# Kloudy-Sky/openintel

Hardware: AMD Instinct MI355X
Metric: queries/sec + p50 latency, 10M-post/768-d hybrid BM25+cosine+RRF top-100 (higher is better)
Workload: dtype f32

## Files before the change

openintel_amd/csrc/api.hip:

```cpp
#include <algorithm>
#include <cstdlib>
#include <cstring>
#include <set>

#include "oi_internal.h"

static thread_local char g_err[512] = "";

void oi_set_error(const char *fmt, ...) {
    va_list ap;
    va_start(ap, fmt);
    vsnprintf(g_err, sizeof(g_err), fmt, ap);
    va_end(ap);
}

__attribute__((constructor)) static void oi_ask_for_more_hw_queues() { (void)setenv("GPU_MAX_HW_QUEUES", "8", 0); }

extern "C" const char *oi_last_error(void) { return g_err; }
extern "C" int oi_abi_version(void) { return OI_ABI_VERSION; }

int oi_dyn_lds(oi_ctx *ctx, const void *kernel, size_t bytes) {
    static std::mutex mu;
    static std::set<std::pair<const void *, int>> done;
    std::lock_guard<std::mutex> g(mu);
    const auto key = std::make_pair(kernel, ctx->device);
    if (done.count(key)) return OI_OK;
    OI_HIP_CHECK(hipFuncSetAttribute(kernel, hipFuncAttributeMaxDynamicSharedMemorySize, (int)bytes));
    done.insert(key);
    return OI_OK;
}

std::atomic<uint64_t> g_oi_ws_epoch{1};

int DevBuf::ensure(size_t bytes) {
    if (bytes <= cap && p) return OI_OK;
    if (borrowed) { oi_set_error("internal: a borrowed buffer cannot grow"); return OI_ERR_STATE; }
    g_oi_ws_epoch.fetch_add(1);
    if (p) {
        (void)hipFree(p);
        p = nullptr;
        cap = 0;
    }
    size_t want = (bytes + 255) & ~(size_t)255;
    if (want == 0) want = 256;
    OI_HIP_CHECK(hipMalloc(&p, want));
    cap = want;
    return OI_OK;
}
void DevBuf::release() {
    if (p) g_oi_ws_epoch.fetch_add(1);
    if (p && !borrowed) (void)hipFree(p);
    p = nullptr;
    cap = 0;
    borrowed = false;
}

int PinBuf::ensure(size_t bytes) {
    if (bytes <= cap) return OI_OK;
    release();
    const size_t want = (bytes + 4095) & ~(size_t)4095;
    if (hipHostMalloc(&p, want, hipHostMallocDefault) == hipSuccess) {
        pinned = true;
    } else {
        (void)hipGetLastError();
        p = aligned_alloc(4096, want);
        pinned = false;
        if (!p) { oi_set_error("host staging buffer: out of memory (%zu bytes)", want); return OI_ERR_HIP; }
    }
    cap = want;
    return OI_OK;
}
void PinBuf::release() {
    if (p) {
        if (pinned) (void)hipHostFree(p);
        else free(p);
    }
    p = nullptr;
    cap = 0;
}

void oi_ctx::prof_begin(const char *tag) {
    ProfSpan s;
    if (hipEventCreateWithFlags(&s.a, hipEventDisableSystemFence) != hipSuccess ||
        hipEventCreateWithFlags(&s.b, hipEventDisableSystemFence) != hipSuccess) return;
    (void)hipEventRecord(s.a, stream);
    prof[tag].push_back(s);
}
void oi_ctx::prof_end(const char *tag) {
    auto it = prof.find(tag);
    if (it == prof.end() || it->second.empty()) return;
    (void)hipEventRecord(it->second.back().b, stream);
}

extern "C" int oi_profile_reset(oi_ctx *ctx, int enable) {
    if (!ctx) { oi_set_error("null ctx"); return OI_ERR_INVALID_ARG; }
    std::lock_guard<std::mutex> g(ctx->mu);
    for (auto &kv : ctx->prof)
        for (auto &s : kv.second) { (void)hipEventDestroy(s.a); (void)hipEventDestroy(s.b); }
    ctx->prof.clear();
    for (const char *runs : {"volume_runs", "summary_runs", "groups_runs", "share_runs"}) {
        auto vr = ctx->ws.find(runs);
        if (vr != ctx->ws.end() && vr->second.p) (void)hipMemsetAsync(vr->second.p, 0, 16, ctx->stream);
    }
    ctx->prof_enabled = enable == 2 ? 2 : (enable != 0 ? 1 : 0);
    return OI_OK;
}

extern "C" int oi_profile_read(oi_ctx *ctx, const char *kernel_tag, double *total_ms_out, uint64_t *launches_out) {
    if (!ctx || !kernel_tag) { oi_set_error("null argument"); return OI_ERR_INVALID_ARG; }
    std::lock_guard<std::mutex> g(ctx->mu);
    OI_HIP_CHECK(hipStreamSynchronize(ctx->stream));
    double total = 0.0;
    uint64_t n = 0;
    if (strncmp(kernel_tag, "flagword", 8) == 0) {
        uint32_t w[4] = {0, 0, 0, 0};
        DevBuf &st = ctx->buf("state_flag");
        if (st.p) OI_HIP_CHECK(hipMemcpy(w, st.p, 16, hipMemcpyDeviceToHost));
        if (total_ms_out) *total_ms_out = (double)w[(kernel_tag[8] - '0') & 3];
        if (launches_out) *launches_out = 0;
        return OI_OK;
    }
    if (strcmp(kernel_tag, "graph_replays") == 0 || strcmp(kernel_tag, "graph_captures") == 0) {
        if (total_ms_out) *total_ms_out = 0.0;
        if (launches_out) *launches_out = kernel_tag[6] == 'r' ? ctx->graph_replays : ctx->graph_captures;
        return OI_OK;
    }
    if (strcmp(kernel_tag, "spec_state") == 0) {
        oi_spec_take_failure(ctx);
        if (total_ms_out) *total_ms_out = (double)ctx->spec_failures;
        if (launches_out) *launches_out = ctx->spec_searches;
        return OI_OK;
    }
    if (strcmp(kernel_tag, "screen_gate") == 0) {
        uint32_t g = 0;
        if (ctx->last_screen_gate) OI_HIP_CHECK(hipMemcpy(&g, ctx->last_screen_gate, 4, hipMemcpyDeviceToHost));
        if (total_ms_out) *total_ms_out = ctx->last_screen_gate ? (double)g : -1.0;
        if (launches_out) *launches_out = 0;
        return OI_OK;
    }
    if (strcmp(kernel_tag, "screen_width") == 0) {
        if (total_ms_out) *total_ms_out = (double)ctx->last_screen_wgs;
        if (launches_out) *launches_out = (uint64_t)ctx->num_cus;
        return OI_OK;
    }
    if (strcmp(kernel_tag, "volume_state") == 0 || strcmp(kernel_tag, "summary_state") == 0 || strcmp(kernel_tag, "groups_state") == 0 ||
        strcmp(kernel_tag, "share_state") == 0) {
        uint32_t w[4] = {0, 0, 0, 0};
        auto vs = ctx->ws.find(kernel_tag);
        if (vs != ctx->ws.end() && vs->second.p) OI_HIP_CHECK(hipMemcpy(w, vs->second.p, 16, hipMemcpyDeviceToHost));
        if (total_ms_out) *total_ms_out = (double)w[2];
        if (launches_out) *launches_out = (w[0] ? 1u : 0u) | (w[1] ? 2u : 0u);
        return OI_OK;
    }
    auto it = ctx->prof.find(kernel_tag);
    if (it != ctx->prof.end())
        for (auto &s : it->second) {
            float ms = 0.f;
            if (hipEventElapsedTime(&ms, s.a, s.b) == hipSuccess) { total += ms; ++n; }
        }
    const char *family = strcmp(kernel_tag, "volume_exact") == 0 ? "volume" : strcmp(kernel_tag, "summary_exact") == 0 ? "summary"
                       : strcmp(kernel_tag, "groups_exact") == 0 ? "groups" : strcmp(kernel_tag, "share_exact") == 0 ? "share" : nullptr;
    if (family) {
        uint32_t runs = 0;
        auto vr = ctx->ws.find(std::string(family) + "_runs");
        if (vr != ctx->ws.end() && vr->second.p) OI_HIP_CHECK(hipMemcpy(&runs, vr->second.p, 4, hipMemcpyDeviceToHost));
        auto fb = ctx->prof.find(std::string(family) + "_fallback");
        if (runs && fb != ctx->prof.end()) {
            for (auto &s : fb->second) {
                float ms = 0.f;
                if (hipEventElapsedTime(&ms, s.a, s.b) == hipSuccess) total += ms;
            }
            n += runs;
        }
    }
    if (total_ms_out) *total_ms_out = total;
    if (launches_out) *launches_out = n;
    return OI_OK;
}

#define OI_MAX_GRAPHS 32

static void graph_free(GraphEntry &e) {
    if (e.exec) (void)hipGraphExecDestroy(e.exec);
    if (e.graph) (void)hipGraphDestroy(e.graph);
    e.exec = nullptr;
    e.graph = nullptr;
}

static void graphs_purge(oi_ctx *ctx, uint64_t index_uid) {
    for (size_t i = 0; i < ctx->graphs.size();)
        if (index_uid == 0 || ctx->graphs[i].key[0] == index_uid) {
            graph_free(ctx->graphs[i]);
            ctx->graphs.erase(ctx->graphs.begin() + (long)i);
        } else ++i;
}

template <class F> static int run_captured(oi_ctx *ctx, const uint64_t (&key)[10], F &&body) {
    if (!ctx->use_graphs || ctx->prof_enabled || !ctx->stream) return body();
    const uint64_t epoch = g_oi_ws_epoch.load();
    GraphEntry *e = nullptr;
    for (auto &g : ctx->graphs)
        if (memcmp(g.key, key, sizeof(key)) == 0) { e = &g; break; }
    if (!e) {
        if (ctx->graphs.size() >= OI_MAX_GRAPHS) {
            size_t lru = 0;
            for (size_t i = 1; i < ctx->graphs.size(); ++i)
                if (ctx->graphs[i].last_use < ctx->graphs[lru].last_use) lru = i;
            OI_HIP_CHECK(hipStreamSynchronize(ctx->stream));
            graph_free(ctx->graphs[lru]);
            ctx->graphs.erase(ctx->graphs.begin() + (long)lru);
        }
        ctx->graphs.emplace_back();
        e = &ctx->graphs.back();
        memcpy(e->key, key, sizeof(key));
        e->last_use = ++ctx->graph_clock;
        const int rc = body();
        e->epoch = g_oi_ws_epoch.load();
        return rc;
    }
    e->last_use = ++ctx->graph_clock;
    if (e->epoch != epoch) {
        OI_HIP_CHECK(hipStreamSynchronize(ctx->stream));
        graph_free(*e);
        e->state = 0;
        const int rc = body();
        e->epoch = g_oi_ws_epoch.load();
        return rc;
    }
    if (e->state == 2) return body();
    if (e->state == 1) {
        OI_HIP_CHECK(hipGraphLaunch(e->exec, ctx->stream));
        ++ctx->graph_replays;
        return OI_OK;
    }
    if (hipStreamBeginCapture(ctx->stream, hipStreamCaptureModeRelaxed) != hipSuccess) {
        (void)hipGetLastError();
        e->state = 2;
        return body();
    }
    const int rc = body();
    hipGraph_t g = nullptr;
    const hipError_t end = hipStreamEndCapture(ctx->stream, &g);
    if (rc != OI_OK || end != hipSuccess || !g || g_oi_ws_epoch.load() != epoch) {
        (void)hipGetLastError();
        if (g) (void)hipGraphDestroy(g);
        e->state = 2;
        if (rc != OI_OK) return rc;
        return body();
    }
    hipGraphExec_t x = nullptr;
    if (hipGraphInstantiate(&x, g, nullptr, nullptr, 0) != hipSuccess || !x) {
        (void)hipGetLastError();
        (void)hipGraphDestroy(g);
        e->state = 2;
        return body();
    }
    e->graph = g;
    e->exec = x;
    e->state = 1;
    ++ctx->graph_captures;
    OI_HIP_CHECK(hipGraphLaunch(e->exec, ctx->stream));
    return OI_OK;
}

extern "C" int oi_set_graph_replay(oi_ctx *ctx, int enable) {
    if (!ctx) { oi_set_error("null ctx"); return OI_ERR_INVALID_ARG; }
    std::lock_guard<std::mutex> g(ctx->mu);
    ctx->use_graphs = enable != 0;
    if (!ctx->use_graphs) {
        OI_HIP_CHECK(hipSetDevice(ctx->device));
        OI_HIP_CHECK(hipStreamSynchronize(ctx->stream));
        graphs_purge(ctx, 0);
    }
    return OI_OK;
}

extern "C" int oi_create(int device_ordinal, oi_ctx **out) {
    if (!out) { oi_set_error("oi_create: out is null"); return OI_ERR_INVALID_ARG; }
    *out = nullptr;
    int n = 0;
    if (hipGetDeviceCount(&n) != hipSuccess || n <= 0) {
        oi_set_error("oi_create: no HIP device visible (this library has no CPU fallback)");
        return OI_ERR_NO_DEVICE;
    }
    OI_REQUIRE(device_ordinal >= 0 && device_ordinal < n, "oi_create: device %d of %d", device_ordinal, n);
    OI_HIP_CHECK(hipSetDevice(device_ordinal));
    hipDeviceProp_t prop;
    OI_HIP_CHECK(hipGetDeviceProperties(&prop, device_ordinal));
    if (strncmp(prop.gcnArchName, "gfx950", 6) != 0) {
        oi_set_error("oi_create: device %d is %s; this library is built for gfx950 only", device_ordinal,
                     prop.gcnArchName);
        return OI_ERR_NO_DEVICE;
    }
    oi_ctx *c = new oi_ctx();
    c->device = device_ordinal;
    c->num_cus = prop.multiProcessorCount > 0 ? prop.multiProcessorCount : 256;
    c->stream = nullptr;
    if (const char *m = getenv("OI_COSINE_MODE"))
        c->cosine_mode = strcmp(m, "split") == 0 ? OI_COSINE_SPLIT : strcmp(m, "exact") == 0 ? OI_COSINE_EXACT
                         : strcmp(m, "screen-copy") == 0 ? OI_COSINE_SCREEN_COPY
                         : strcmp(m, "screen-stream") == 0 ? OI_COSINE_SCREEN_STREAM : OI_COSINE_SCREEN;
    if (hipEventCreateWithFlags(&c->ev_fork, hipEventDisableTiming) != hipSuccess) c->ev_fork = nullptr;
    if (hipEventCreateWithFlags(&c->ev_join, hipEventDisableTiming) != hipSuccess) c->ev_join = nullptr;
    *out = c;
    return OI_OK;
}

extern "C" int oi_create_like(oi_ctx *like, oi_ctx **out) {
    if (!out) { oi_set_error("oi_create_like: out is null"); return OI_ERR_INVALID_ARG; }
    *out = nullptr;
    if (!like) { oi_set_error("null ctx"); return OI_ERR_INVALID_ARG; }
    OI_CHECK(oi_create(like->device, out));
    std::lock_guard<std::mutex> g(like->mu);
    (*out)->cosine_mode = like->cosine_mode;
    (*out)->overlap_legs = like->overlap_legs;
    (*out)->speculate = like->speculate;
    (*out)->use_graphs = like->use_graphs;
    return OI_OK;
}

static void ctx_release(oi_ctx *ctx) {
    if (ctx->refs.fetch_sub(1) != 1) return;
    (void)hipSetDevice(ctx->device);
    if (ctx->side_stream) { (void)hipStreamSynchronize(ctx->side_stream); (void)hipStreamDestroy(ctx->side_stream); }
    if (ctx->ev_fork) (void)hipEventDestroy(ctx->ev_fork);
    if (ctx->ev_join) (void)hipEventDestroy(ctx->ev_join);
    oi_profile_reset(ctx, 0);
    graphs_purge(ctx, 0);
    for (auto &kv : ctx->ws) kv.second.release();
    ctx->pin_in.release();
    ctx->pin_out.release();
    if (ctx->spec_fail_host) (void)hipHostFree(ctx->spec_fail_host);
    delete ctx;
}

extern "C" void oi_destroy(oi_ctx *ctx) {
    if (!ctx) return;
    {
        std::lock_guard<std::mutex> g(ctx->mu);
        (void)hipSetDevice(ctx->device);
        (void)hipStreamSynchronize(ctx->stream);
        if (ctx->refs.load() > 1) ctx->stream = nullptr;
    }
    ctx_release(ctx);
}

extern "C" int oi_workspace_bytes(oi_ctx *ctx, uint64_t *device_bytes, uint64_t *pinned_bytes) {
    if (!ctx) { oi_set_error("null ctx"); return OI_ERR_INVALID_ARG; }
    std::lock_guard<std::mutex> g(ctx->mu);
    uint64_t d = 0;
    for (auto &kv : ctx->ws)
        if (!kv.second.borrowed) d += kv.second.cap;
    if (device_bytes) *device_bytes = d;
    if (pinned_bytes) *pinned_bytes = (ctx->pin_in.pinned ? ctx->pin_in.cap : 0) + (ctx->pin_out.pinned ? ctx->pin_out.cap : 0);
    return OI_OK;
}

extern "C" int oi_set_stream(oi_ctx *ctx, void *hip_stream) {
    if (!ctx) { oi_set_error("null ctx"); return OI_ERR_INVALID_ARG; }
    std::lock_guard<std::mutex> g(ctx->mu);
    ctx->stream = reinterpret_cast<hipStream_t>(hip_stream);
    return OI_OK;
}

extern "C" int oi_set_cosine_mode(oi_ctx *ctx, int mode) {
    if (!ctx) { oi_set_error("null ctx"); return OI_ERR_INVALID_ARG; }
    OI_REQUIRE(mode == OI_COSINE_EXACT || mode == OI_COSINE_SPLIT || mode == OI_COSINE_SCREEN || mode == OI_COSINE_SCREEN_COPY ||
                   mode == OI_COSINE_SCREEN_STREAM,
               "oi_set_cosine_mode: unknown mode %d", mode);
    std::lock_guard<std::mutex> g(ctx->mu);
    ctx->cosine_mode = mode;
    return OI_OK;
}

extern "C" int oi_set_overlap(oi_ctx *ctx, int enable) {
    if (!ctx) { oi_set_error("null ctx"); return OI_ERR_INVALID_ARG; }
    std::lock_guard<std::mutex> g(ctx->mu);
    ctx->overlap_legs = enable != 0;
    return OI_OK;
}

extern "C" int oi_set_screen_speculation(oi_ctx *ctx, int enable) {
    if (!ctx) { oi_set_error("null ctx"); return OI_ERR_INVALID_ARG; }
    std::lock_guard<std::mutex> g(ctx->mu);
    ctx->speculate = enable != 0;
    ctx->spec_skip = ctx->spec_backoff = 0;
    return OI_OK;
}

static int check_overflow_locked(oi_ctx *ctx) {
    DevBuf &st = ctx->buf("state_flag");
    if (!st.p) return OI_OK;
    uint32_t f = 0;
    OI_HIP_CHECK(hipMemcpyAsync(&f, st.p, sizeof(f), hipMemcpyDeviceToHost, ctx->stream));
    OI_HIP_CHECK(hipStreamSynchronize(ctx->stream));
    if (f) {
        OI_HIP_CHECK(hipMemsetAsync(st.p, 0, 16, ctx->stream));
        oi_set_error("internal candidate pool overflowed");
        return OI_ERR_OVERFLOW;
    }
    return OI_OK;
}

extern "C" int oi_synchronize(oi_ctx *ctx) {
    if (!ctx) { oi_set_error("null ctx"); return OI_ERR_INVALID_ARG; }
    std::lock_guard<std::mutex> g(ctx->mu);
    OI_HIP_CHECK(hipSetDevice(ctx->device));
    OI_HIP_CHECK(hipStreamSynchronize(ctx->stream));
    return check_overflow_locked(ctx);
}

extern "C" int oi_lexicon_analyze_device(oi_ctx *ctx, const uint8_t *d_blob, const uint64_t *d_offsets,
                                         uint64_t n, uint64_t blob_bytes, double *d_pol, uint8_t *d_spec) {
    if (!ctx) { oi_set_error("null ctx"); return OI_ERR_INVALID_ARG; }
    if (n == 0) return OI_OK;
    OI_REQUIRE(d_offsets && d_pol && d_spec && (d_blob || blob_bytes == 0), "lexicon: null buffer");
    std::lock_guard<std::mutex> g(ctx->mu);
    OI_HIP_CHECK(hipSetDevice(ctx->device));
    return oi_launch_lexicon(ctx, d_blob, d_offsets, n, blob_bytes, d_pol, d_spec);
}

extern "C" int oi_lexicon_summary_device(oi_ctx *ctx, const uint8_t *d_blob, const uint64_t *d_offsets, uint64_t n,
                                         uint64_t blob_bytes, const uint8_t *d_sources, double tau, double *d_pol,
                                         uint8_t *d_spec, oi_social_counters *out) {
    if (!ctx || !out) { oi_set_error("null argument"); return OI_ERR_INVALID_ARG; }
    if (n == 0) { memset(out, 0, sizeof(*out)); return OI_OK; }
    OI_REQUIRE(d_offsets && (d_blob || blob_bytes == 0), "lexicon summary: null buffer");
    std::lock_guard<std::mutex> g(ctx->mu);
    OI_HIP_CHECK(hipSetDevice(ctx->device));
    return oi_launch_lexicon_fused(ctx, d_blob, d_offsets, n, blob_bytes, d_pol, d_spec, d_sources, tau, out);
}

extern "C" int oi_lexicon_analyze(oi_ctx *ctx, const uint8_t *blob, const uint64_t *offsets, uint64_t n,
                                  double *pol_out, uint8_t *spec_out) {
    if (!ctx) { oi_set_error("null ctx"); return OI_ERR_INVALID_ARG; }
    if (n == 0) return OI_OK;
    OI_REQUIRE(offsets && pol_out && spec_out, "lexicon: null buffer");
    OI_REQUIRE(offsets[0] == 0, "lexicon: offsets[0] must be 0");
    const uint64_t bytes = offsets[n];
    OI_REQUIRE(blob || bytes == 0, "lexicon: null text blob");
    std::lock_guard<std::mutex> g(ctx->mu);
    OI_HIP_CHECK(hipSetDevice(ctx->device));
    hipStream_t st = ctx->stream;
    const size_t off_o = (bytes + 15) & ~(size_t)15, in_bytes = off_o + sizeof(uint64_t) * (n + 1);
    const size_t out_bytes = sizeof(double) * n + n;
// ... 1620 lines not shown
```

openintel_amd/csrc/cosine_screen_i8.hip:

```cpp
#include <algorithm>
#include <cmath>
#include <cstdlib>
#include <type_traits>

#include "oi_device.h"
#include "oi_internal.h"
#include "oi_screen_stage.h"
#include "oi_lds_dma.h"

typedef int i8s_i32x4 __attribute__((ext_vector_type(4)));
typedef int i8s_i32x16 __attribute__((ext_vector_type(16)));
typedef float i8s_f32x2 __attribute__((ext_vector_type(2)));
template <int N>
struct i8s_ivec {
    typedef int type __attribute__((ext_vector_type(N)));
};

#define I8S_TILE_ROWS 32
#define I8S_SLOT_BYTES (I8S_TILE_ROWS * 128)
#define I8S_META_BYTES 256
#define I8S_PAD_ROWS 64

size_t oi_screen_i8_meta_offset(uint64_t n, uint32_t dim) { return ((size_t)n * dim + 255) & ~(size_t)255; }
size_t oi_screen_i8_bytes(uint64_t n, uint32_t dim) {
    return oi_screen_i8_meta_offset(n, dim) + 8 * ((size_t)n + I8S_PAD_ROWS) + 256;
}

__global__ __launch_bounds__(256) void i8s_make_kernel(const float *__restrict__ rows, uint64_t n, uint32_t dim,
                                                       const uint32_t *__restrict__ long_bitmap, uint32_t *__restrict__ out_i8,
                                                       float *__restrict__ meta, uint32_t *__restrict__ emax_bits) {
    const uint32_t lane = threadIdx.x & 63;
    const uint64_t wave = ((uint64_t)blockIdx.x * blockDim.x + threadIdx.x) >> 6;
    const uint64_t n_waves = ((uint64_t)gridDim.x * blockDim.x) >> 6;
    const uint32_t nv = dim >> 2;
    float best = 0.f;
    for (uint64_t r = wave; r < n; r += n_waves) {
        const float4 *x = reinterpret_cast<const float4 *>(rows + r * dim);
        float4 v[3];
        float amax = 0.f;
#pragma unroll
        for (int u = 0; u < 3; ++u) {
            const uint32_t j = lane + 64u * u;
            v[u] = j < nv ? x[j] : make_float4(0.f, 0.f, 0.f, 0.f);
            amax = fmaxf(amax, fmaxf(fmaxf(fabsf(v[u].x), fabsf(v[u].y)), fmaxf(fabsf(v[u].z), fabsf(v[u].w))));
        }
#pragma unroll
        for (int o = 32; o > 0; o >>= 1) amax = fmaxf(amax, __shfl_xor(amax, o, OI_WAVE));
        const float s = amax / 127.f;
        double e2 = 0.0;
#pragma unroll
        for (int u = 0; u < 3; ++u) {
            const uint32_t j = lane + 64u * u;
            const float xs[4] = {v[u].x, v[u].y, v[u].z, v[u].w};
            uint32_t packed = 0;
#pragma unroll
            for (int c = 0; c < 4; ++c) {
                float t = s > 0.f ? rintf(xs[c] / s) : 0.f;
                t = fminf(127.f, fmaxf(-127.f, t));
                const int iv = (int)t;
                const double e = (double)s * (double)iv - (double)xs[c];
                e2 += j < nv ? e * e : 0.0;
                packed |= ((uint32_t)iv & 0xFFu) << (8 * c);
            }
            if (j < nv) out_i8[r * nv + j] = packed;
        }
        e2 = oi_wave_sum(e2);
        const float er = (float)sqrt(e2) * 1.00000095367431640625f;
        if (lane == 0) {
            meta[2 * r] = s;
            meta[2 * r + 1] = er;
        }
        const bool is_long = long_bitmap && ((long_bitmap[r >> 5] >> (r & 31)) & 1u);
        if (!is_long) best = fmaxf(best, er);
    }
    if (lane == 0) atomicMax(emax_bits, __float_as_uint(best));
}

int oi_launch_make_screen_i8(oi_ctx *ctx, const float *rows, uint64_t n, uint32_t dim, const uint32_t *long_bitmap, uint8_t *out) {
    OI_REQUIRE(oi_cosine_screen_supported(dim), "int8 screening copy: dim %u not instantiated (384, 768)", dim);
    const size_t mo = oi_screen_i8_meta_offset(n, dim);
    OI_HIP_CHECK(hipMemsetAsync(out + mo, 0, 8 * ((size_t)n + I8S_PAD_ROWS) + 256, ctx->stream));
    if (n == 0) return OI_OK;
    uint64_t blocks = (n + 3) / 4;
    const uint64_t cap = (uint64_t)ctx->num_cus * 8;
    if (blocks > cap) blocks = cap;
    float *meta = reinterpret_cast<float *>(out + mo);
    hipLaunchKernelGGL(i8s_make_kernel, dim3((uint32_t)blocks), dim3(256), 0, ctx->stream, rows, n, dim, long_bitmap,
                       reinterpret_cast<uint32_t *>(out), meta, reinterpret_cast<uint32_t *>(meta + 2 * (n + I8S_PAD_ROWS)));
    OI_HIP_CHECK(hipGetLastError());
    return OI_OK;
}

#define I8S_NORM_LIMIT 1.0e15f
#define I8S_QNORM_MIN 1.0e-12f
__device__ __forceinline__ void i8s_stage_query_row(const float *__restrict__ q, uint32_t row, uint32_t n_queries, uint32_t n_padded, uint32_t dim,
                                                    const uint32_t *__restrict__ max_norm_bits, const uint32_t *__restrict__ emax_bits,
                                                    int8_t *__restrict__ qi8, float *__restrict__ qf, uint32_t *gate) {
    const uint32_t lane = threadIdx.x & 63;
    const bool real = row < n_queries;
    float amax = 0.f;
    bool fin = true;
    for (uint32_t k = lane; k < dim; k += 64) {
        const float f = real ? q[(uint64_t)row * dim + k] : 0.f;
        fin = fin && (f - f == 0.f);
        amax = fmaxf(amax, fabsf(f));
    }
#pragma unroll
    for (int o = 32; o > 0; o >>= 1) amax = fmaxf(amax, __shfl_xor(amax, o, OI_WAVE));
    fin = __builtin_amdgcn_ballot_w64(!fin) == 0ull;
    const float a = fin ? amax / 127.f : 0.f;
    double qn2 = 0.0, en2 = 0.0;
    for (uint32_t k = lane; k < dim; k += 64) {
        const float f = real ? q[(uint64_t)row * dim + k] : 0.f;
        float h = 0.f, l = 0.f;
        if (a > 0.f) {
            const float t = f / a;
            h = fminf(127.f, fmaxf(-127.f, rintf(t)));
            l = fminf(127.f, fmaxf(-127.f, rintf((t - h) * 128.f)));
        }
        const double qh = (double)a * ((double)h + (double)l * 0.0078125);
        qn2 += qh * qh;
        en2 += (qh - (double)f) * (qh - (double)f);
        qi8[(uint64_t)row * dim + k] = (int8_t)(int)h;
        qi8[((uint64_t)n_padded + row) * dim + k] = (int8_t)(int)l;
    }
    qn2 = oi_wave_sum(qn2);
    en2 = oi_wave_sum(en2);
    if (lane == 0) {
        const float up = 1.00000095367431640625f;
        const float qn = (float)sqrt(qn2) * up, en = (float)sqrt(en2) * up;
        const float X = __uint_as_float(max_norm_bits[0]), em = __uint_as_float(*emax_bits);
        const bool ok = fin && amax > 0.f && qn < I8S_NORM_LIMIT && qn >= I8S_QNORM_MIN && X < I8S_NORM_LIMIT && em < I8S_NORM_LIMIT;
        const float rnd = 3.814697265625e-06f + (float)dim * 2.384185791015625e-07f;
        const float cq = 1.001f * (X * en + rnd * (X + em) * (qn + en)) + 1.0e-27f;
        const float m2 = 2.002f * (em * qn + cq);
        qf[row] = ok ? a : 0.f;
        qf[n_padded + row] = ok ? qn : 0.f;
        qf[2 * n_padded + row] = ok ? cq : 0.f;
        qf[3 * n_padded + row] = ok || !real ? m2 : __builtin_inff();
        if (real && !ok) *gate = 1u;
    }
}
__global__ __launch_bounds__(256) void i8s_stage_kernel(const float *__restrict__ q, uint32_t n_queries, uint32_t n_padded, uint32_t dim,
                                                        const uint32_t *__restrict__ max_norm_bits, const uint32_t *__restrict__ emax_bits,
                                                        int8_t *__restrict__ qi8, float *__restrict__ qf, uint32_t *gate) {
    const uint32_t wave = (blockIdx.x * blockDim.x + threadIdx.x) >> 6, n_waves = (gridDim.x * blockDim.x) >> 6;
    for (uint32_t row = wave; row < n_padded; row += n_waves) {
        i8s_stage_query_row(q, row, n_queries, n_padded, dim, max_norm_bits, emax_bits, qi8, qf, gate);
    }
}

__global__ __launch_bounds__(256) void i8s_stage_both_kernel(const float *__restrict__ q, uint32_t n_queries, uint32_t n_padded, uint32_t dim,
                                                             const uint32_t *__restrict__ max_norm_bits, const uint32_t *__restrict__ emax_bits,
                                                             int8_t *__restrict__ qi8, float *__restrict__ qf, uint16_t *__restrict__ q_bf16,
                                                             float *__restrict__ eps2, uint32_t *gate) {
    const uint32_t wave = (blockIdx.x * blockDim.x + threadIdx.x) >> 6, n_waves = (gridDim.x * blockDim.x) >> 6;
    for (uint32_t row = wave; row < n_padded; row += n_waves) {
        i8s_stage_query_row(q, row, n_queries, n_padded, dim, max_norm_bits, emax_bits, qi8, qf, gate);
        pf_stage_query_row(q, row, n_queries, dim, max_norm_bits, q_bf16, eps2, gate);
    }
}

int oi_launch_screen_stage_i8(oi_ctx *ctx, const float *d_queries, uint32_t n_queries, uint32_t dim, const uint32_t *max_norm_bits,
                              const uint8_t *i8_copy, uint64_t n_rows, int8_t *qi8, float *qf, uint32_t *gate, uint16_t *q_bf16,
                              float *eps2) {
    const uint32_t n_padded = (n_queries + 31u) & ~31u;
    if (n_padded == 0) return OI_OK;
    const uint32_t *emax = reinterpret_cast<const uint32_t *>(i8_copy + oi_screen_i8_meta_offset(n_rows, dim)) + 2 * (n_rows + I8S_PAD_ROWS);
    if (q_bf16)
        hipLaunchKernelGGL(i8s_stage_both_kernel, dim3((n_padded + 3) / 4), dim3(256), 0, ctx->stream, d_queries, n_queries, n_padded, dim,
                           max_norm_bits, emax, qi8, qf, q_bf16, eps2, gate);
    else
        hipLaunchKernelGGL(i8s_stage_kernel, dim3((n_padded + 3) / 4), dim3(256), 0, ctx->stream, d_queries, n_queries, n_padded, dim,
                           max_norm_bits, emax, qi8, qf, gate);
    OI_HIP_CHECK(hipGetLastError());
    return OI_OK;
}

__device__ __forceinline__ void i8s_issue_piece(const oi_u32x4 &srd, uint32_t voff, uint32_t soff, uint32_t lds_dst) {
#ifdef I8S_NO_DMA
    (void)srd; (void)voff; (void)soff; (void)lds_dst;
#else
    oi_dma_piece(srd, voff, soff, lds_dst);
#endif
}
__device__ __forceinline__ void i8s_issue_meta(const oi_u32x4 &srd, uint32_t voff, uint32_t lds_dst) {
#ifdef I8S_NO_DMA
    (void)srd; (void)voff; (void)lds_dst;
#else
    uint32_t keep;
    const uint32_t d = __builtin_amdgcn_readfirstlane(lds_dst);
    asm volatile(
        "s_mov_b32 %0, m0\n\t"
        "s_mov_b32 m0, %3\n\t"
        "s_nop 0\n\t"
        "buffer_load_dword %1, %2, 0 offen " OI_DMA_NT "lds\n\t"
        "s_mov_b32 m0, %0"
        : "=&s"(keep)
        : "v"(voff), "s"(srd), "s"(d)
        : "memory");
#endif
}

template <int D, int NQT, int NBUF, bool FILT>
__global__ __launch_bounds__(256, 1) void cosine_i8_screen(
    const uint8_t *__restrict__ rows, const float *__restrict__ meta, uint64_t row_begin, uint64_t row_end,
    const int8_t *__restrict__ qhi, const int8_t *__restrict__ qlo,
    const float *__restrict__ qf, uint32_t qf_stride, uint32_t n_queries, uint32_t doc_id_base, uint64_t *pools, uint32_t *seg_cnt,
    uint32_t seg_cnt_stride, const uint32_t *tau_keys, uint64_t pool_stride, uint32_t carry_cap, uint32_t seg_cap, uint32_t *overflow,
    const uint4 *__restrict__ filt, const uint2 *__restrict__ attrs) {
    constexpr int NKC = D / 128;
    constexpr int P = NBUF - 1;
    constexpr int KSTEPS = D / 32;
    constexpr uint32_t RING = NBUF * I8S_SLOT_BYTES;
    static_assert(D % 128 == 0 && P >= 2 && P <= 2 * NKC, "unsupported ring depth for this D");
    constexpr uint32_t QLO_LDS = NQT * KSTEPS * 64 * 16;
    static_assert(NQT * KSTEPS * 4 <= 200, "the hi query block must fit the register file");
    static_assert(4 * RING + 4 * 2 * I8S_META_BYTES + 256 + OI_STAGE_LDS + QLO_LDS <= 160 * 1024, "LDS");

    extern __shared__ __attribute__((aligned(1024))) unsigned char smem[];
    unsigned char *ring = smem;
    unsigned char *meta_lds = smem + 4 * RING;
    uint32_t *seg_fill = reinterpret_cast<uint32_t *>(smem + 4 * RING + 8 * I8S_META_BYTES);
    unsigned char *stage_base = smem + 4 * RING + 8 * I8S_META_BYTES + 256;
    unsigned char *qlo_lds = stage_base + OI_STAGE_LDS;

    OI_CLAIM_WHOLE_SIMD();
    const uint32_t tid = threadIdx.x, lane = tid & 63;
    const uint32_t w = __builtin_amdgcn_readfirstlane(tid >> 6);
    const uint32_t li = lane & 31, lh = lane >> 5;
    uint64_t *stage_keys = reinterpret_cast<uint64_t *>(stage_base) + w * OI_STAGE;
    uint32_t *stage_q = reinterpret_cast<uint32_t *>(stage_base + 4 * OI_STAGE * 8) + w * OI_STAGE;
    uint32_t st_head = 0, st_n = 0;

    i8s_i32x4 qh[NQT][KSTEPS];
#pragma unroll
    for (int t = 0; t < NQT; ++t)
#pragma unroll
        for (int s = 0; s < KSTEPS; ++s)
            qh[t][s] = *reinterpret_cast<const i8s_i32x4 *>(qhi + (uint64_t)(32 * t + li) * D + 32 * s + 16 * lh);
    for (uint32_t c = tid; c < (uint32_t)(NQT * KSTEPS * 64); c += 256) {
        const uint32_t t = c / (KSTEPS * 64), s = (c / 64) % KSTEPS, l = c % 64;
        *reinterpret_cast<i8s_i32x4 *>(qlo_lds + c * 16) =
            *reinterpret_cast<const i8s_i32x4 *>(qlo + (uint64_t)(32 * t + (l & 31)) * D + 32 * s + 16 * (l >> 5));
    }
    float qa[NQT], qn[NQT], cq[NQT], tc[NQT];
#pragma unroll
    for (int t = 0; t < NQT; ++t) {
        const uint32_t q = 32u * t + li;
        const bool real = q < n_queries;
        const uint32_t k = real ? tau_keys[q] : 0xFFFFFFFFu;
        const float tau = k <= 0x007FFFFFu ? -__builtin_inff() : oi_key_f32(k);
        qa[t] = real ? qf[q] * 0.0078125f : 0.f;
        qn[t] = real ? qf[qf_stride + q] : 0.f;
        cq[t] = real ? qf[2 * qf_stride + q] : 0.f;
        const float m2 = real ? qf[3 * qf_stride + q] : 0.f;
        const float T = m2 < __builtin_inff() ? (tau + m2) - (fabsf(tau) + m2) * 9.5367431640625e-07f : -__builtin_inff();
        tc[t] = T - cq[t];
    }
    if (tid < 32 * NQT) seg_fill[tid] = 0;
#ifdef I8S_NO_DMA
    for (uint32_t i = tid; i < (4 * RING + 8 * I8S_META_BYTES) / 4; i += 256) reinterpret_cast<uint32_t *>(smem)[i] = 0u;
#endif
    __syncthreads();

    const uint64_t n_rows = row_end - row_begin;
    const uint64_t n_tiles = (n_rows + I8S_TILE_ROWS - 1) / I8S_TILE_ROWS;
    const uint64_t first = (uint64_t)blockIdx.x * 4 + w, stride = (uint64_t)gridDim.x * 4;
    const uint64_t my_nt = first < n_tiles ? (n_tiles - first + stride - 1) / stride : 0;
    uint64_t *my_seg = pools + carry_cap + (uint64_t)blockIdx.x * seg_cap;

    if (my_nt) {
        uint32_t voff[4];
#pragma unroll
        for (int m = 0; m < 4; ++m) {
            const uint32_t prow = 8 * m + (lane >> 3);
            voff[m] = prow * (uint32_t)D + (((lane & 7) ^ ((prow >> 1) & 7)) << 4);
        }
        const uint32_t ring_w = oi_lds_addr(ring) + w * RING;
        const unsigned char *ring_rd = ring + w * RING;
        const uint32_t meta_w = oi_lds_addr(meta_lds) + w * 2 * I8S_META_BYTES;
        const unsigned char *meta_rd = meta_lds + w * 2 * I8S_META_BYTES;
        uint32_t frag_off[4];
#pragma unroll
        for (int g = 0; g < 4; ++g) frag_off[g] = li * 128 + (((2 * g + lh) ^ ((li >> 1) & 7)) << 4);

        auto tile_row0 = [&](uint64_t ti) { return row_begin + (first + ti * stride) * (uint64_t)I8S_TILE_ROWS; };
        auto tile_srd = [&](uint64_t ti) {
            const uint64_t r0 = tile_row0(ti < my_nt ? ti : 0);
            return oi_make_srd(rows + r0 * D, ti < my_nt ? (row_end - r0) * (uint64_t)D : 0ull);
        };
        auto issue_meta = [&](uint64_t ti) {
            const uint64_t r0 = tile_row0(ti);
            i8s_issue_meta(oi_make_srd(meta + 2 * r0, (row_end - r0) * 8ull), lane * 4u, meta_w + (uint32_t)(ti & 1) * I8S_META_BYTES);
        };
        oi_u32x4 s0 = tile_srd(0), s1 = tile_srd(1), s2 = tile_srd(2);
        __builtin_amdgcn_s_waitcnt(0x0F70);
        oi_static_for<0, P>([&](auto j_) {
            constexpr int j = decltype(j_)::value;
            constexpr int tj = j / NKC, kj = j % NKC;
#pragma unroll
            for (int m = 0; m < 4; ++m)
                i8s_issue_piece(tj == 0 ? s0 : (tj == 1 ? s1 : s2), voff[m], kj * 128, ring_w + j * I8S_SLOT_BYTES + m * 1024);
        });
        issue_meta(0);
        uint32_t rd_off = 0, wr_off = (NBUF - 1) * I8S_SLOT_BYTES;
        auto lo_frag = [&](int t, int s) {
            return *reinterpret_cast<const i8s_i32x4 *>(qlo_lds + ((t * KSTEPS + s) * 64 + lane) * 16);
        };
        i8s_i32x4 b_cur[NQT];
#ifndef I8S_NO_MFMA
#pragma unroll
        for (int t = 0; t < NQT; ++t) b_cur[t] = lo_frag(t, 0);
#endif

        oi_wait_vm<4 * (P - 1)>();
        i8s_i32x4 a_cur = *reinterpret_cast<const i8s_i32x4 *>(ring_rd + frag_off[0]);

        constexpr int NS = 16 * NQT;
        constexpr int RPK = KSTEPS >= 20 ? 1 : 2;
        constexpr int NSL = 16 / RPK, T0 = 4;
        static_assert(T0 + NSL <= KSTEPS, "the tile test does not fit the span");
        static_assert(4 * NKC + 4 >= 4 * (P - 1) - 1, "the ring's wait in k-step 3 must retire the previous tile's metadata");
        typename i8s_ivec<NS>::type S;
#pragma unroll
        for (int i = 0; i < NS; ++i) S[i] = 0;
        i8s_i32x16 ah[NQT], al[NQT];
        i8s_f32x2 md_cur[RPK];
#pragma unroll
        for (int u = 0; u < RPK; ++u) md_cur[u] = i8s_f32x2{0.f, 0.f};
        const uint32_t lh32 = 32u * lh;
        auto meta_row = [&](const unsigned char *mt, int r) {
            return *reinterpret_cast<const i8s_f32x2 *>(mt + lh32 + ((r & 3) + 8 * (r >> 2)) * 8);
        };
        float cap_sc = 0.f, cap_er = 0.f;
        auto test_row = [&](int t, int r, const i8s_f32x2 md) -> uint32_t {
            const float sc = oi_mul_unpacked((float)S[16 * t + r], oi_mul_unpacked(md[0], qa[t]));
            const bool pass = sc >= oi_fma_unpacked(-md[1], qn[t], tc[t]);
            cap_sc = pass ? sc : cap_sc;
            cap_er = pass ? md[1] : cap_er;
            return pass ? 1u << (16 * t + r) : 0u;
        };

        for (uint64_t ti = 0;; ++ti) {
            const bool live = ti < my_nt;
            const unsigned char *mt = meta_rd + (uint32_t)((ti + 1) & 1) * I8S_META_BYTES;
            uint32_t m = 0;
            if (live) {
#pragma unroll
                for (int t = 0; t < NQT; ++t)
#pragma unroll
                    for (int r = 0; r < 16; ++r) { ah[t][r] = 0; al[t][r] = 0; }

                oi_static_for<0, NKC * 4>([&](auto gi_) {
                    constexpr int gi = decltype(gi_)::value;
                    constexpr int kc = gi / 4, g = gi % 4;
                    constexpr int sn = kc + P;
                    constexpr int tn = sn / NKC, kn = sn % NKC;
                    i8s_i32x4 a_nxt;
                    if constexpr (g < 3) {
                        a_nxt = *reinterpret_cast<const i8s_i32x4 *>(ring_rd + rd_off + frag_off[g + 1]);
                    } else {
                        oi_wait_vm<4 * (P - 1) - 1>();
                        const uint32_t nx_off = rd_off + I8S_SLOT_BYTES == RING ? 0u : rd_off + I8S_SLOT_BYTES;
                        a_nxt = *reinterpret_cast<const i8s_i32x4 *>(ring_rd + nx_off + frag_off[0]);
                    }
                    i8s_f32x2 md_nxt[RPK];
                    if constexpr (gi >= T0 - 1 && gi < T0 - 1 + NSL) {
#pragma unroll
                        for (int u = 0; u < RPK; ++u) md_nxt[u] = meta_row(mt, RPK * (gi - (T0 - 1)) + u);
                    }
#ifndef I8S_NO_MFMA
                    i8s_i32x4 b_nxt[NQT];
#pragma unroll
                    for (int t = 0; t < NQT; ++t) b_nxt[t] = lo_frag(t, (gi + 1) % KSTEPS);
#endif
                    __builtin_amdgcn_sched_barrier(0);
#pragma unroll
                    for (int t = 0; t < NQT; ++t) {
#ifndef I8S_NO_MFMA
                        ah[t] = __builtin_amdgcn_mfma_i32_32x32x32_i8(a_cur, qh[t][gi], ah[t], 0, 0, 0);
                        al[t] = __builtin_amdgcn_mfma_i32_32x32x32_i8(a_cur, b_cur[t], al[t], 0, 0, 0);
#else
                        asm volatile("" : : "v"(a_cur));
#endif
                        if constexpr (gi >= T0 && gi < T0 + NSL) if (t == 0) {
#pragma unroll
                            for (int u = 0; u < RPK; ++u)
#pragma unroll
                                for (int tt = 0; tt < NQT; ++tt) m |= test_row(tt, RPK * (gi - T0) + u, md_cur[u]);
                            asm volatile("" : "+v"(m), "+v"(cap_sc), "+v"(cap_er));
                        }
                        __builtin_amdgcn_sched_barrier(0);
                    }
#ifndef I8S_NO_MFMA
#pragma unroll
                    for (int t = 0; t < NQT; ++t) b_cur[t] = b_nxt[t];
#endif
                    if constexpr (gi >= T0 - 1 && gi < T0 - 1 + NSL) {
#pragma unroll
                        for (int u = 0; u < RPK; ++u) md_cur[u] = md_nxt[u];
                    }
                    i8s_issue_piece(tn == 0 ? s0 : (tn == 1 ? s1 : s2), voff[g], kn * 128, ring_w + wr_off + g * 1024);
                    if constexpr (g == 3) {
                        wr_off = rd_off;
                        rd_off = rd_off + I8S_SLOT_BYTES == RING ? 0u : rd_off + I8S_SLOT_BYTES;
                    }
                    a_cur = a_nxt;
                });
            } else {
                oi_wait_vm<0>();
#pragma unroll
                for (int r = 0; r < 16; ++r) {
                    const i8s_f32x2 md = meta_row(mt, r);
#pragma unroll
                    for (int t = 0; t < NQT; ++t) m |= test_row(t, r, md);
                }
            }

            const uint64_t row0 = tile_row0(ti ? ti - 1 : 0);
            if (ti == 0) m = 0u;
            const uint32_t m_tested = m;
            if (row_end - row0 < (uint64_t)I8S_TILE_ROWS) {
                const uint32_t left = (uint32_t)(row_end - row0);
#pragma unroll
                for (int r = 0; r < 16; ++r)
                    if ((uint32_t)((r & 3) + 8 * (r >> 2)) + 4u * lh >= left) m &= ~(0x00010001u << r);
            }
#if defined(I8S_NO_DMA) || defined(I8S_NO_MFMA) || defined(I8S_NO_APPEND)
            if (seg_cap != 0xFFFFFFFFu) m = 0u;
#endif
            if (__builtin_amdgcn_ballot_w64(m != 0u) != 0ull) {
                if constexpr (FILT) m = oi_filter_tile<NQT>(m, filt, attrs, row0, lh, li);
                static_assert(64u <= OI_STAGE - OI_STAGE_FLUSH, "a tile of one pair per lane must fit the staging ring");
                if (__builtin_amdgcn_ballot_w64((m_tested & (m_tested - 1u)) != 0u) == 0ull) {
                    const uint64_t has = __builtin_amdgcn_ballot_w64(m != 0u);
                    if (m != 0u) {
                        const uint32_t bit = (uint32_t)__builtin_ctz(m), r = bit & 15u;
                        const bool t1 = NQT > 1 && bit >= 16u;
                        const uint32_t rit = (r & 3) + 8 * (r >> 2) + 4 * lh;
                        const float low = cap_sc - fmaf(cap_er, t1 ? qn[NQT - 1] : qn[0], t1 ? cq[NQT - 1] : cq[0]);
                        const uint32_t below = __builtin_amdgcn_mbcnt_hi((uint32_t)(has >> 32), __builtin_amdgcn_mbcnt_lo((uint32_t)has, 0u));
                        const uint32_t idx = (st_head + st_n + below) & (OI_STAGE - 1);
                        stage_keys[idx] = oi_rank_key(low, doc_id_base + ((uint32_t)row0 + rit));
                        stage_q[idx] = (t1 ? 32u : 0u) + li;
                    }
                    st_n += (uint32_t)__builtin_popcountll(has);
                    while (st_n >= OI_STAGE_FLUSH) {
                        OI_STAGE_FLUSH_TO_POOL(OI_STAGE_FLUSH);
                    }
                } else {
                    const uint32_t cnt = (uint32_t)__builtin_popcount(m);
                    const uint32_t incl = oi_wave_incl_scan(cnt);
                    const uint32_t total = (uint32_t)__builtin_amdgcn_readlane((int)incl, 63);
                    const uint32_t any = oi_wave_or(m);
                    auto lower_key = [&](int t, uint32_t r) -> uint64_t {
                        const uint32_t rit = (r & 3) + 8 * (r >> 2) + 4 * lh;
                        const i8s_f32x2 md = *reinterpret_cast<const i8s_f32x2 *>(mt + rit * 8);
                        const float sc = (float)S[16 * t + r] * (md[0] * qa[t]);
                        return oi_rank_key(sc - fmaf(md[1], qn[t], cq[t]), doc_id_base + ((uint32_t)row0 + rit));
                    };
                    if (total <= OI_STAGE - OI_STAGE_FLUSH) {
                        uint32_t idx = st_head + st_n + incl - cnt;
#pragma unroll
                        for (int t = 0; t < NQT; ++t)
                            for (uint32_t wd = (any >> (16 * t)) & 0xFFFFu; wd; wd &= wd - 1) {
                                const uint32_t r = (uint32_t)__builtin_ctz(wd);
                                if (m & (1u << (16 * t + r))) {
                                    stage_keys[idx & (OI_STAGE - 1)] = lower_key(t, r);
                                    stage_q[idx & (OI_STAGE - 1)] = 32u * t + li;
                                    ++idx;
                                }
                            }
                        st_n += total;
                        while (st_n >= OI_STAGE_FLUSH) {
                            OI_STAGE_FLUSH_TO_POOL(OI_STAGE_FLUSH);
                        }
                    } else {
                        uint32_t pos[NQT];
#pragma unroll
                        for (int t = 0; t < NQT; ++t)
                            pos[t] = atomicAdd(&seg_fill[32u * t + li], (uint32_t)__builtin_popcount((m >> (16 * t)) & 0xFFFFu));
#pragma unroll
                        for (int t = 0; t < NQT; ++t) {
                            uint64_t *dst = my_seg + (uint64_t)(32u * t + li) * pool_stride;
                            for (uint32_t wd = (any >> (16 * t)) & 0xFFFFu; wd; wd &= wd - 1) {
                                const uint32_t r = (uint32_t)__builtin_ctz(wd);
                                if (m & (1u << (16 * t + r))) {
                                    if (pos[t] < seg_cap) dst[pos[t]] = lower_key(t, r);
                                    else *overflow = 1u;
                                    ++pos[t];
                                }
                            }
                        }
                    }
                }
            }
            if (!live) break;
#pragma unroll
            for (int t = 0; t < NQT; ++t)
#pragma unroll
                for (int r = 0; r < 16; ++r) S[16 * t + r] = ah[t][r] * 128 + al[t][r];
            if (ti + 1 < my_nt) issue_meta(ti + 1);
            s0 = s1;
            s1 = s2;
            s2 = tile_srd(ti + 3);
        }
        if (st_n) {
            OI_STAGE_FLUSH_TO_POOL(st_n);
        }
        oi_wait_vm<0>();
    }
    __syncthreads();
    if (tid < 32 * NQT && tid < n_queries) {
        const uint32_t c = seg_fill[tid];
        seg_cnt[(uint64_t)tid * seg_cnt_stride + blockIdx.x] = c < seg_cap ? c : seg_cap;
    }
}

template <int D, int NQT, int NBUF, bool FILT>
static int launch_i8_screen_k(oi_ctx *ctx, const uint8_t *rows, const float *meta, uint64_t row_begin, uint64_t row_end, const int8_t *qhi,
                              const int8_t *qlo, const float *qf, uint32_t qf_stride, uint32_t nq, uint32_t doc_id_base, const PoolView &p) {
    constexpr size_t smem = 4 * NBUF * I8S_SLOT_BYTES + 8 * I8S_META_BYTES + 256 + OI_STAGE_LDS + NQT * (D / 32) * 64 * 16;
    OI_CHECK(oi_dyn_lds(ctx, reinterpret_cast<const void *>(cosine_i8_screen<D, NQT, NBUF, FILT>), (size_t)(smem)));
    hipLaunchKernelGGL((cosine_i8_screen<D, NQT, NBUF, FILT>), dim3(p.n_segs), dim3(256), smem, ctx->stream, rows, meta, row_begin, row_end,
                       qhi, qlo, qf, qf_stride, nq, doc_id_base, p.keys, p.seg_cnt, p.seg_cnt_stride, p.tau_keys, p.stride, p.carry_cap,
                       p.seg_cap, p.overflow, p.filt, p.attrs);
    OI_HIP_CHECK(hipGetLastError());
    return OI_OK;
}
template <int D, int NQT, int NBUF>
static int launch_i8_screen(oi_ctx *ctx, const uint8_t *rows, const float *meta, uint64_t row_begin, uint64_t row_end, const int8_t *qhi,
                            const int8_t *qlo, const float *qf, uint32_t qf_stride, uint32_t nq, uint32_t doc_id_base, const PoolView &p) {
    return p.filt ? launch_i8_screen_k<D, NQT, NBUF, true>(ctx, rows, meta, row_begin, row_end, qhi, qlo, qf, qf_stride, nq, doc_id_base, p)
                  : launch_i8_screen_k<D, NQT, NBUF, false>(ctx, rows, meta, row_begin, row_end, qhi, qlo, qf, qf_stride, nq, doc_id_base, p);
}

int oi_launch_cosine_screen_i8_chunk(oi_ctx *ctx, const uint8_t *i8_copy, uint64_t n_rows_total, uint64_t row_begin, uint64_t row_end,
                                     uint32_t dim, const int8_t *qi8, const float *qf, uint32_t n_queries, uint32_t doc_id_base,
                                     PoolView &pool, uint32_t wgs) {
    OI_REQUIRE(oi_cosine_screen_supported(dim), "cosine screen (int8): dim %u not instantiated (384, 768)", dim);
    OI_REQUIRE(row_end <= n_rows_total, "cosine screen (int8): rows past the copy");
    const uint64_t chunk_rows = row_end > row_begin ? row_end - row_begin : 0;
    if (wgs) oi_cosine_screen_geometry(ctx, chunk_rows, wgs, &pool.n_segs, &pool.seg_cap);
    else oi_cosine_screen_geometry(ctx, chunk_rows, &pool.n_segs, &pool.seg_cap);
    OI_REQUIRE(pool.n_segs <= pool.seg_cnt_stride && pool.carry_cap + (uint64_t)pool.n_segs * pool.seg_cap <= pool.stride,
               "cosine screen (int8): chunk does not fit the candidate pool");
    if (row_end <= row_begin || n_queries == 0) return OI_OK;
    const float *meta = reinterpret_cast<const float *>(i8_copy + oi_screen_i8_meta_offset(n_rows_total, dim));
    const uint32_t np = (n_queries + 31u) & ~31u;
    ProfScope ps(ctx, "cosine");
    for (uint32_t q0 = 0; q0 < n_queries; q0 += 64) {
        const uint32_t nq_here = std::min(64u, n_queries - q0);
        const PoolView p = pool.for_queries(q0);
        const int8_t *qhi = qi8 + (uint64_t)q0 * dim, *qlo = qi8 + ((uint64_t)np + q0) * dim;
        const float *qfp = qf + q0;
        const bool two = nq_here > 32;
        if (dim == 768) {
            if (two) OI_CHECK((launch_i8_screen<768, 2, 6>(ctx, i8_copy, meta, row_begin, row_end, qhi, qlo, qfp, np, nq_here, doc_id_base, p)));
            else OI_CHECK((launch_i8_screen<768, 1, 6>(ctx, i8_copy, meta, row_begin, row_end, qhi, qlo, qfp, np, nq_here, doc_id_base, p)));
        } else {
            if (two) OI_CHECK((launch_i8_screen<384, 2, 6>(ctx, i8_copy, meta, row_begin, row_end, qhi, qlo, qfp, np, nq_here, doc_id_base, p)));
            else OI_CHECK((launch_i8_screen<384, 1, 6>(ctx, i8_copy, meta, row_begin, row_end, qhi, qlo, qfp, np, nq_here, doc_id_base, p)));
        }
    }
    return OI_OK;
}

__device__ __forceinline__ float i8s_bf16_lo(uint32_t w) { return __uint_as_float(w << 16); }
__device__ __forceinline__ float i8s_bf16_hi(uint32_t w) { return __uint_as_float(w & 0xFFFF0000u); }
__global__ __launch_bounds__(256) void pf_rescreen_kernel(const uint16_t *__restrict__ copy, uint64_t n_rows, uint32_t dim,
                                                          uint32_t doc_id_base, const uint16_t *__restrict__ qb, uint64_t *pools,
                                                          const uint32_t *__restrict__ cnt, uint64_t stride, uint32_t cap) {
    const uint32_t q = blockIdx.y, lane = threadIdx.x & 63;
    const uint32_t wave = (blockIdx.x * blockDim.x + threadIdx.x) >> 6, n_waves = (gridDim.x * blockDim.x) >> 6;
    uint32_t c = cnt[q];
    c = c < cap ? c : cap;
    uint64_t *keys = pools + (uint64_t)q * stride;
    const uint32_t nvec = dim >> 3;
    const uint4 *qv = reinterpret_cast<const uint4 *>(qb + (uint64_t)q * dim);
    for (uint32_t i0 = wave * 4u; i0 < c; i0 += n_waves * 4u) {
        uint32_t doc[4];
        const uint4 *x[4];
        float a[4];
#pragma unroll
        for (int u = 0; u < 4; ++u) {
            const uint32_t i = i0 + u < c ? i0 + u : c - 1u;
            doc[u] = oi_rank_key_doc(keys[i]);
            const uint64_t r = (uint64_t)(doc[u] - doc_id_base);
            x[u] = reinterpret_cast<const uint4 *>(copy + (r < n_rows ? r : 0) * dim);
            a[u] = 0.f;
        }
        for (uint32_t v = lane; v < nvec; v += 64) {
            const uint4 yv = qv[v];
            uint4 xv[4];
#pragma unroll
            for (int u = 0; u < 4; ++u) xv[u] = oi_load_stream(x[u] + v);
#pragma unroll
            for (int u = 0; u < 4; ++u) {
                const uint32_t xw[4] = {xv[u].x, xv[u].y, xv[u].z, xv[u].w}, yw[4] = {yv.x, yv.y, yv.z, yv.w};
#pragma unroll
                for (int e = 0; e < 4; ++e) {
                    a[u] = oi_fma_unpacked(i8s_bf16_lo(xw[e]), i8s_bf16_lo(yw[e]), a[u]);
                    a[u] = oi_fma_unpacked(i8s_bf16_hi(xw[e]), i8s_bf16_hi(yw[e]), a[u]);
                }
            }
        }
        float s[4];
#pragma unroll
        for (int u = 0; u < 4; ++u) s[u] = oi_wave_sum(a[u]);
#pragma unroll
        for (int u = 0; u < 4; ++u) {
            const uint64_t r = (uint64_t)(doc[u] - doc_id_base);
            const float sc = r < n_rows ? s[u] : 0.f;
            if (lane == 0 && i0 + u < c) keys[i0 + u] = oi_rank_key(sc, doc[u]);
        }
    }
}

int oi_launch_rescreen_bf16(oi_ctx *ctx, const uint16_t *copy_rows, uint64_t n_rows, uint32_t dim, uint32_t doc_id_base,
                            const uint16_t *q_bf16, uint32_t n_queries, const PoolView &pool) {
    if (n_queries == 0) return OI_OK;
    ProfScope ps(ctx, "rescreen");
    hipLaunchKernelGGL(pf_rescreen_kernel, dim3(32, n_queries), dim3(256), 0, ctx->stream, copy_rows, n_rows, dim, doc_id_base, q_bf16,
                       pool.keys, pool.carry_cnt, pool.stride, pool.carry_cap);
    OI_HIP_CHECK(hipGetLastError());
    return OI_OK;
}
```

openintel_amd/csrc/oi_internal.h:

```cpp
#pragma once

#include <hip/hip_runtime.h>

#include <cstdarg>
#include <cstdint>
#include <cstdio>
#include <cstdlib>
#include <cstring>
#include <atomic>
#include <map>
#include <mutex>
#include <string>
#include <utility>
#include <vector>

#include "openintel_hip.h"

void oi_set_error(const char *fmt, ...);

#define OI_HIP_CHECK(expr)                                                                   \
    do {                                                                                     \
        hipError_t oi_e_ = (expr);                                                           \
        if (oi_e_ != hipSuccess) {                                                           \
            oi_set_error("%s failed: %s (%s:%d)", #expr, hipGetErrorString(oi_e_), __FILE__, \
                         __LINE__);                                                          \
            return OI_ERR_HIP;                                                               \
        }                                                                                    \
    } while (0)

#define OI_CHECK(expr)              \
    do {                            \
        int oi_rc_ = (expr);        \
        if (oi_rc_ != OI_OK) return oi_rc_; \
    } while (0)

#define OI_REQUIRE(cond, ...)         \
    do {                              \
        if (!(cond)) {                \
            oi_set_error(__VA_ARGS__); \
            return OI_ERR_INVALID_ARG; \
        }                             \
    } while (0)

struct oi_ctx;
int oi_dyn_lds(oi_ctx *ctx, const void *kernel, size_t bytes);

#ifdef OI_ABLATION
inline const char *oi_ablation_env(const char *name) { return getenv(name); }
#else
inline const char *oi_ablation_env(const char *) { return nullptr; }
#endif

struct DevBuf {
    void *p = nullptr;
    size_t cap = 0;
    bool borrowed = false;
    DevBuf() = default;
    DevBuf(const DevBuf &) = delete;
    DevBuf &operator=(const DevBuf &) = delete;
    ~DevBuf() { release(); }
    int ensure(size_t bytes);
    void release();
    template <class T> T *as() const { return reinterpret_cast<T *>(p); }
};

#define OI_PINNED_STAGE_MAX ((size_t)1 << 20)
struct PinBuf {
    void *p = nullptr;
    size_t cap = 0;
    bool pinned = false;
    PinBuf() = default;
    PinBuf(const PinBuf &) = delete;
    PinBuf &operator=(const PinBuf &) = delete;
    int ensure(size_t bytes);
    void release();
    template <class T> T *as() const { return reinterpret_cast<T *>(p); }
};

struct ProfSpan {
    hipEvent_t a, b;
};

extern std::atomic<uint64_t> g_oi_ws_epoch;

struct GraphEntry {
    uint64_t key[10] = {0, 0, 0, 0, 0, 0, 0, 0, 0, 0};
    uint64_t epoch = 0, last_use = 0;
    int state = 0;
    hipGraph_t graph = nullptr;
    hipGraphExec_t exec = nullptr;
};

struct oi_ctx {
    std::atomic<int> refs{1};
    int device = 0;
    int num_cus = 256;
    hipStream_t stream = nullptr;
    hipStream_t side_stream = nullptr;
    bool side_stream_failed = false;
    hipEvent_t ev_fork = nullptr, ev_join = nullptr;
    bool overlap_legs = true;
    bool speculate = true;
    uint32_t spec_skip = 0, spec_backoff = 0;
    uint32_t *spec_fail_host = nullptr;
    uint64_t spec_searches = 0, spec_failures = 0;
    int cosine_mode = 2;
    std::mutex mu;
    std::map<std::string, DevBuf> ws;
    int prof_enabled = 0;
    const uint32_t *run_gate = nullptr;
    const uint32_t *last_screen_gate = nullptr;
    uint32_t last_screen_wgs = 0;
    std::map<std::string, std::vector<ProfSpan>> prof;
    std::vector<hipEvent_t> event_pool;
    bool use_graphs = false;
    std::vector<GraphEntry> graphs;
    uint64_t graph_clock = 0, graph_replays = 0, graph_captures = 0;

    PinBuf pin_in, pin_out;

    DevBuf &buf(const char *name) { return ws[name]; }
    void prof_begin(const char *tag);
    void prof_end(const char *tag);
};

struct ProfScope {
    oi_ctx *c;
    const char *tag;
    bool on;
    ProfScope(oi_ctx *ctx, const char *t) : c(ctx), tag(t) {
        on = c->prof_enabled == 1 || (c->prof_enabled == 2 && strcmp(t, "cosine") == 0);
        if (on) c->prof_begin(tag);
    }
    ~ProfScope() {
        if (on) c->prof_end(tag);
    }
};

#define OI_BM25_FLOOR_RANKS 4
struct oi_index {
    uint64_t uid = 0;
    std::atomic<int> refs{1};
    oi_index *src = nullptr;
    oi_ctx *ctx = nullptr;
    uint64_t n_docs = 0;
    uint32_t dim = 0, vocab = 0, doc_id_base = 0;

    float *rows = nullptr;
    bool rows_owned = false;
    uint16_t *rows_bf16 = nullptr;
    bool rows_bf16_owned = false;
    DevBuf max_row_norm;
    bool screen_ok = false;
    uint32_t n_long = 0;
    DevBuf long_list, long_bitmap;
    DevBuf screen_copy;
    int screen_copy_policy = -1;
    DevBuf screen_i8;
    DevBuf doc_attrs;
    DevBuf signals;

    bool forward_set = false, finalized = false;
    uint64_t total_tokens = 0;
    uint64_t n_postings = 0;
    uint32_t n_blocks = 0;
    uint32_t n_win = 0;
    DevBuf uniq_keys;
    DevBuf tf;
    DevBuf doc_len;
    DevBuf df_local;

    DevBuf postings;
    DevBuf cell_start;
    DevBuf idf;
    DevBuf impact_floor;
    DevBuf fwd_terms;
    DevBuf fwd_offsets;
    float avgdl = 0.f;
    uint32_t max_query_terms = 16;
    int bm25_mode = 0;
    bool is_view = false;
};

int search_lists_device(oi_index *idx, const float *d_qv, const uint32_t *d_qt, const uint32_t *d_qo, uint32_t B, uint32_t depth,
                        float *cos_s, uint32_t *cos_d, uint32_t *cos_c, float *bm_s, uint32_t *bm_d, uint32_t *bm_c,
                        const uint4 *d_filt = nullptr, const uint2 *d_attrs = nullptr);
void oi_spec_take_failure(oi_ctx *ctx);

int oi_launch_lexicon(oi_ctx *ctx, const uint8_t *d_blob, const uint64_t *d_offsets, uint64_t n,
                      uint64_t blob_bytes, double *d_pol, uint8_t *d_spec);
int oi_launch_lexicon_fused(oi_ctx *ctx, const uint8_t *d_blob, const uint64_t *d_offsets, uint64_t n, uint64_t blob_bytes,
                            double *d_pol, uint8_t *d_spec, const uint8_t *d_sources, double tau, oi_social_counters *summary);
int oi_launch_social_summary(oi_ctx *ctx, const uint8_t *d_sources, const double *d_pol,
                             const uint8_t *d_spec, uint64_t n, double tau,
                             oi_social_counters *out_host);
int oi_launch_social_summary_segmented(oi_ctx *ctx, const uint8_t *d_sources, const double *d_pol, const uint8_t *d_spec,
                                       uint64_t n, const uint64_t *d_seg, uint64_t n_seg, double tau,
                                       oi_social_counters *d_out);
int oi_launch_headline_scan(oi_ctx *ctx, const uint8_t *d_blob, const uint64_t *d_offsets, uint64_t n,
                            uint64_t blob_bytes, const uint8_t *ticker, uint64_t ticker_len,
                            const uint8_t *forms_blob, const uint32_t *form_offsets, uint32_t n_forms,
                            uint16_t *d_mask, uint64_t *d_order, uint8_t *d_about);
size_t oi_headline_params_bytes();
int oi_headline_build_params(void *dst, const uint8_t *ticker, uint64_t ticker_len, const uint8_t *forms_blob,
                             const uint32_t *form_offsets, uint32_t n_forms);
int oi_launch_headline_scan_params(oi_ctx *ctx, const uint8_t *d_blob, const uint64_t *d_offsets, uint64_t n,
                                   uint64_t blob_bytes, uint64_t text_bytes, const void *d_params, uint16_t *d_mask,
                                   uint64_t *d_order, uint8_t *d_about);
struct PoolView {
    uint64_t *keys;
    uint32_t *carry_cnt;
    uint32_t *seg_cnt;
    uint32_t *tau_keys;
    uint64_t stride;
    uint32_t carry_cap;
    uint32_t seg_cap;
    uint32_t n_segs;
    uint32_t seg_cnt_stride;
    uint32_t *overflow;
    const uint4 *filt = nullptr;
    const uint2 *attrs = nullptr;

    PoolView for_queries(uint32_t q0) const {
        PoolView p = *this;
        p.keys += (uint64_t)q0 * stride;
        p.carry_cnt += q0;
        p.seg_cnt += (uint64_t)q0 * seg_cnt_stride;
        if (p.tau_keys) p.tau_keys += q0;
        if (p.filt) p.filt += q0;
        return p;
    }
};
struct SelectExtra {
    const float *eps2 = nullptr;
    uint32_t *margin_gate = nullptr;
    const uint32_t *run_gate = nullptr;
    const uint32_t *skip_bitmap = nullptr;
    uint32_t skip_base = 0;
    uint64_t *cand = nullptr;
    uint32_t cand_cap = 0;
    const float *row_meta = nullptr;
    uint32_t meta_base = 0;
    const float *row_qn = nullptr, *row_cq = nullptr;
    uint32_t spec_rank = 0;
    uint32_t *spec_tau = nullptr, *spec_max = nullptr;
};
int oi_launch_select(oi_ctx *ctx, const PoolView &pool, uint32_t n_queries, uint32_t k, bool compact,
                     float *out_scores, uint32_t *out_docs, uint32_t *out_counts, uint32_t out_stride,
                     const SelectExtra *extra = nullptr);
int oi_launch_lists_to_pool(oi_ctx *ctx, const float *scores, const uint32_t *docs,
                            const uint32_t *counts, uint64_t shard_stride, uint64_t count_stride,
                            uint32_t n_shards, uint32_t n_queries, uint32_t depth, const PoolView &pool);
int oi_launch_rrf(oi_ctx *ctx, const uint32_t *docs_a, const uint32_t *counts_a, const uint32_t *docs_b,
                  const uint32_t *counts_b, uint32_t n_queries, uint32_t depth, uint32_t k,
                  float *scores_out, uint32_t *docs_out, uint32_t *counts_out);
int oi_launch_collapse(oi_index *idx, const float *d_scores, const uint32_t *d_docs, const uint32_t *d_counts, uint32_t n_queries,
                       uint32_t depth, float threshold, uint32_t k, float *scores_out, uint32_t *docs_out, uint32_t *counts_out,
                       uint32_t *dup_out);
int oi_launch_similar_volume(oi_index *idx, const float *d_q, uint32_t n_queries, const oi_volume_spec &spec, const uint4 *d_filt,
                             uint32_t *d_counts);
int oi_launch_volume_round_queries(oi_ctx *ctx, const float *d_q, uint64_t total, float *d_out);
int oi_launch_pack_signals(oi_ctx *ctx, const double *d_pol, const uint8_t *d_spec, const uint8_t *d_sources, uint64_t n, double tau,
                           uint2 *d_out);
int oi_launch_similar_summary(oi_index *idx, const float *d_q, uint32_t n_queries, const oi_summary_spec &spec, const float *d_thresholds,
                              const uint4 *d_filt, oi_social_counters *d_out);
int oi_launch_similar_groups(oi_index *idx, const float *d_q, uint32_t n_queries, const oi_groups_spec &spec, const float *d_thresholds,
                             const uint4 *d_filt, oi_social_counters *d_records, uint32_t *d_keys, uint32_t *d_counts,
                             uint32_t *d_qualified);
int oi_launch_similar_share(oi_index *idx, const float *d_q, uint32_t n_queries, const oi_summary_spec &spec, const float *d_thresholds,
                            const uint4 *d_filt, oi_social_counters *d_out, uint32_t *d_labels);
int oi_launch_mention_summary(oi_index *idx, const uint32_t *d_terms, const uint32_t *d_offsets, uint32_t n_queries,
                              const oi_mention_spec &spec, const uint32_t *d_min_match, const uint4 *d_filt, oi_social_counters *d_out);
int oi_launch_label_sums(oi_index *idx, const uint32_t *d_labels, uint32_t n_clusters, int64_t *d_sums, uint64_t *d_counts);
int oi_launch_centroids_from_sums(oi_ctx *ctx, const int64_t *d_sums, const uint64_t *d_counts, const float *d_previous,
                                  uint32_t n_clusters, uint32_t dim, float *d_out);
int oi_launch_fit_moved(oi_ctx *ctx, const uint32_t *d_cur, const uint32_t *d_prev, uint64_t n, uint64_t *d_out);
int oi_launch_cosine_chunk(oi_ctx *ctx, const float *rows, uint64_t row_begin, uint64_t row_end,
                           uint32_t dim, const float *d_queries_padded, uint32_t n_queries,
                           uint32_t n_queries_padded, uint32_t doc_id_base, PoolView &pool);
uint64_t oi_cosine_max_chunk_rows(const oi_ctx *ctx, uint32_t dim, uint32_t n_queries, uint64_t stride,
                                  uint32_t carry_cap);
int oi_launch_l2_normalize(oi_ctx *ctx, float *rows, uint64_t n, uint32_t dim);
bool oi_cosine_split_supported(uint32_t dim);
int oi_launch_cosine_split(oi_ctx *ctx, const float *rows, uint64_t row_begin, uint64_t row_end, uint32_t dim,
                           const float *d_queries, uint32_t nq, uint32_t doc_id_base, const PoolView &p);
bool oi_cosine_bf16_supported(uint32_t dim);
int oi_launch_cosine_bf16_chunk(oi_ctx *ctx, const uint16_t *rows, uint64_t row_begin, uint64_t row_end, uint32_t dim,
                                const float *d_queries, uint32_t n_queries, uint32_t doc_id_base, PoolView &pool);
uint32_t oi_cosine_query_padding(uint32_t n_queries);
bool oi_cosine_ksplit_supported(uint32_t dim);
bool oi_cosine_screen_supported(uint32_t dim);
inline bool oi_index_screenable(const oi_index *idx) {
    return idx->rows && !idx->rows_bf16 && idx->screen_ok && oi_cosine_screen_supported(idx->dim);
}
void oi_cosine_screen_geometry(const oi_ctx *ctx, uint64_t n_rows, uint32_t *n_segs, uint32_t *seg_cap);
void oi_cosine_screen_geometry(const oi_ctx *ctx, uint64_t n_rows, uint32_t wgs, uint32_t *n_segs, uint32_t *seg_cap);
int oi_launch_row_norm_max(oi_ctx *ctx, const float *rows, uint64_t n, uint32_t dim, uint32_t *max_bits);
int oi_launch_screen_stage(oi_ctx *ctx, const float *d_queries, uint32_t n_queries, uint32_t dim,
                           const uint32_t *max_norm_bits, uint16_t *q_bf16, float *eps2, uint32_t *gate);
int oi_launch_cosine_screen_chunk(oi_ctx *ctx, const float *rows, uint64_t row_begin, uint64_t row_end, uint32_t dim,
                                  const uint16_t *q_bf16, uint32_t n_queries, uint32_t doc_id_base, PoolView &pool);
int oi_launch_make_screen_copy(oi_ctx *ctx, const float *rows, uint64_t n, uint32_t dim, uint16_t *out);
#define OI_I8_CARRY 16384u
size_t oi_screen_i8_bytes(uint64_t n, uint32_t dim);
size_t oi_screen_i8_meta_offset(uint64_t n, uint32_t dim);
int oi_launch_make_screen_i8(oi_ctx *ctx, const float *rows, uint64_t n, uint32_t dim, const uint32_t *long_bitmap, uint8_t *out);
int oi_launch_screen_stage_i8(oi_ctx *ctx, const float *d_queries, uint32_t n_queries, uint32_t dim, const uint32_t *max_norm_bits,
                              const uint8_t *i8_copy, uint64_t n_rows, int8_t *qi8, float *qf, uint32_t *gate,
                              uint16_t *q_bf16 = nullptr, float *eps2 = nullptr);
int oi_launch_cosine_screen_i8_chunk(oi_ctx *ctx, const uint8_t *i8_copy, uint64_t n_rows_total, uint64_t row_begin, uint64_t row_end,
                                     uint32_t dim, const int8_t *qi8, const float *qf, uint32_t n_queries, uint32_t doc_id_base,
                                     PoolView &pool, uint32_t wgs = 0);
int oi_launch_rescreen_bf16(oi_ctx *ctx, const uint16_t *copy_rows, uint64_t n_rows, uint32_t dim, uint32_t doc_id_base,
                            const uint16_t *q_bf16, uint32_t n_queries, const PoolView &pool);
int oi_launch_cosine_screen_copy_chunk(oi_ctx *ctx, const uint16_t *copy_rows, uint64_t row_begin, uint64_t row_end, uint32_t dim,
                                       const uint16_t *q_bf16, uint32_t n_queries, uint32_t doc_id_base, PoolView &pool);
int oi_launch_screen_probe(oi_ctx *ctx, const float *rows, uint64_t row_begin, uint32_t n_rows, uint32_t dim,
                           const uint16_t *q_bf16, uint32_t n_queries, float *d_out);
int oi_launch_spec_threshold(oi_ctx *ctx, const PoolView &pool, uint32_t n_queries, uint32_t r, const float *eps2, uint32_t *spec_tau,
                             uint32_t *spec_max);
int oi_launch_spec_compare(oi_ctx *ctx, uint32_t n_queries, const uint32_t *tau_a, const uint32_t *max_a, const uint32_t *tau_b,
                           const uint32_t *max_b);
int oi_launch_rescore(oi_ctx *ctx, const float *rows, uint64_t n_rows, uint32_t dim, uint32_t doc_id_base,
                      const float *d_queries, uint32_t n_queries, const PoolView &in, const PoolView &out,
                      const uint32_t *extra_docs = nullptr, uint32_t n_extra = 0, const uint32_t *spec_max = nullptr,
                      const uint32_t *tau_final = nullptr, uint32_t *gate = nullptr, uint32_t *fail_host = nullptr);
#define OI_LONG_ROWS_MAX 1024u
int oi_launch_row_norm_classes(oi_ctx *ctx, const float *rows, uint64_t n, uint32_t dim, float X0, float E0, uint32_t *cls,
                               uint32_t *bitmap, uint32_t *list, uint32_t cap);
int oi_launch_cosine_ksplit(oi_ctx *ctx, const float *rows, uint64_t row_begin, uint64_t row_end, uint32_t dim,
                            const float *q, uint32_t nq, bool two_tiles, uint32_t doc_id_base, const PoolView &p);
int oi_bm25_stage_forward(oi_index *idx, const uint32_t *d_terms, const uint64_t *d_offsets);
int oi_bm25_finalize(oi_index *idx, uint64_t global_n, uint64_t global_tokens, const uint32_t *global_df_host);
void oi_bm25_scan_geometry(const oi_ctx *ctx, uint64_t n_docs, uint32_t *n_segs, uint32_t *seg_cap);
uint32_t oi_bm25_scan_pass_queries(uint32_t max_terms_per_query);
int oi_launch_bm25_scan(oi_index *idx, const uint32_t *d_q_terms, const uint32_t *d_q_offsets, uint32_t q_begin,
                        uint32_t nq, uint64_t doc_begin, uint64_t doc_end, float avgdl, bool run_setup,
                        const PoolView &pool);
uint32_t oi_bm25_wave_pass_queries(void);
int oi_launch_bm25_wave(oi_index *idx, const uint32_t *d_q_terms, const uint32_t *d_q_offsets, uint32_t q_begin,
                        uint32_t nq, const PoolView &pool, uint32_t block_begin, uint32_t block_end);
uint32_t oi_bm25_stream_pass_queries(void);
uint32_t oi_bm25_stream_seg_cap(uint32_t depth, bool first_phase);
int oi_launch_bm25_plan(oi_index *idx, const uint32_t *d_q_terms, const uint32_t *d_q_offsets, uint32_t q_begin, uint32_t nq,
                        uint32_t *state, uint64_t state_words, uint32_t depth, uint32_t tau_off, uint32_t tau_words, bool with_floors);
int oi_launch_bm25_stream(oi_index *idx, const uint32_t *d_q_terms, const uint32_t *d_q_offsets, uint32_t q_begin,
                          uint32_t nq, uint32_t depth, const PoolView &pool, uint32_t block_begin, uint32_t block_end);
int oi_launch_bm25(oi_index *idx, const uint32_t *d_q_terms, const uint32_t *d_q_offsets,
                   uint32_t n_queries, uint32_t depth, const PoolView &pool, uint32_t block_begin,
                   uint32_t block_end);

struct oi_comm {
    oi_ctx *ctx = nullptr;
    void *nccl = nullptr;
    uint32_t rank = 0, world = 1;
};
int oi_rccl_unique_id(uint8_t *id_out);
int oi_rccl_init(void **comm_out, uint32_t world, const uint8_t *id_bytes, uint32_t rank);
void oi_rccl_destroy(void *comm);
int oi_rccl_all_gather_u32(void *comm, const uint32_t *send, uint32_t *recv, size_t words, hipStream_t st);
int oi_rccl_all_reduce_sum(void *comm, void *buf, size_t count, bool u64, hipStream_t st);
```

openintel_amd/csrc/search.hip:

```cpp
#include <algorithm>

#include "oi_internal.h"

namespace {

int env_int(const char *name, int dflt, int lo) { return oi_ablation_env(name) ? std::max(lo, atoi(oi_ablation_env(name))) : dflt; }
bool env_set(const char *name) { return oi_ablation_env(name) != nullptr; }
struct Knobs {
    uint64_t first_mult = env_int("OI_FIRST_CHUNK_MULT", 1, 1), first_div = env_int("OI_FIRST_CHUNK_DIV", 1, 1);
    uint64_t growth = env_int("OI_CHUNK_GROWTH", 0, 2);
    uint64_t spec_growth = env_int("OI_SPEC_GROWTH", 128, 2), spec_first_div = env_int("OI_SPEC_FIRST_DIV", 4, 1);
    uint32_t bm25_first_div = env_int("OI_BM25_FIRST_DIV", 8, 1);
    bool screen_no_round = env_set("OI_SCREEN_NO_ROUND"), no_spec = env_set("OI_NO_SPEC"), no_overlap = env_set("OI_NO_OVERLAP");
    bool bm25_beside_last = env_set("OI_BM25_BESIDE_LAST"), screen_i8_narrow = env_set("OI_SCREEN_I8_NARROW");
    bool bm25_early = env_set("OI_BM25_EARLY"), small_gemv = env_set("OI_SMALL_BATCH_GEMV"), bm25_two_phase = env_set("OI_BM25_TWO_PHASE");
    bool exact_only = env_set("OI_COSINE_V1") || env_set("OI_SELECT_V1");
};
const Knobs &knobs() { static const Knobs k; return k; }

struct Pools { PoolView cos, bm; };
enum { BM25_TAAT = 1, BM25_SCAN = 2, BM25_WAVE = 3, BM25_STREAM = 4 };
int bm25_mode_of(const oi_index *idx) {
    static const char *mode_env = getenv("OI_BM25_MODE");
    int mode = idx->bm25_mode;
    if (mode == 0 && mode_env)
        mode = strcmp(mode_env, "scan") == 0 ? 2 : strcmp(mode_env, "taat") == 0 ? 1 : strcmp(mode_env, "wave") == 0 ? 3 : 4;
    return mode == 0 ? 4 : mode;
}
int prepare_pools(oi_ctx *ctx, uint32_t B, uint64_t cos_alloc_stride, uint64_t cos_stride, uint32_t carry_cap, uint32_t bm_blocks,
                  uint32_t depth, Pools *out, size_t extra_words, uint32_t **extra) {
    DevBuf &flag = ctx->buf("state_flag");
    if (!flag.p) {
        OI_CHECK(flag.ensure(16));
        OI_HIP_CHECK(hipMemsetAsync(flag.p, 0, 16, ctx->stream));
    }
    const uint32_t cos_segs = (uint32_t)ctx->num_cus * (B <= 8 ? 8u : 1u);
    const uint32_t bm_segs = bm_blocks ? bm_blocks : 1;
    const size_t words = (size_t)B * (2 + cos_segs + 2 + bm_segs);
    DevBuf &st = ctx->buf("pool_state");
    OI_CHECK(st.ensure(sizeof(uint32_t) * (words + extra_words)));
    OI_HIP_CHECK(hipMemsetAsync(st.p, 0, sizeof(uint32_t) * (words + extra_words), ctx->stream));
    *extra = st.as<uint32_t>() + words;
    const uint64_t bm_stride = (uint64_t)carry_cap + (uint64_t)bm_segs * depth;
    DevBuf &pc = ctx->buf("pool_cos"), &pb = ctx->buf("pool_bm");
    OI_CHECK(pc.ensure(sizeof(uint64_t) * (size_t)B * cos_alloc_stride));
    OI_CHECK(pb.ensure(sizeof(uint64_t) * (size_t)B * bm_stride));
    uint32_t *s = st.as<uint32_t>();
    uint32_t *cos_carry = s, *cos_tau = s + B, *cos_seg = s + 2 * (size_t)B;
    uint32_t *bm_carry = cos_seg + (size_t)B * cos_segs, *bm_tau = bm_carry + B, *bm_seg = bm_tau + B;
    out->cos = PoolView{pc.as<uint64_t>(), cos_carry, cos_seg, cos_tau, cos_stride, carry_cap, 0, 0, cos_segs, flag.as<uint32_t>()};
    out->bm = PoolView{pb.as<uint64_t>(), bm_carry, bm_seg, bm_tau, bm_stride, carry_cap, depth, bm_segs, bm_segs, flag.as<uint32_t>()};
    return OI_OK;
}

uint64_t oi_first_chunk_rows(uint32_t depth) {
    return std::max<uint64_t>(std::max<uint64_t>(8192, 32ull * depth) * knobs().first_mult / knobs().first_div, 2ull * depth);
}
uint64_t oi_screen_first_chunk_rows(const oi_ctx *ctx, uint32_t depth) {
    uint64_t rows = oi_first_chunk_rows(depth);
    const uint64_t round = 32ull * 4 * std::max<uint64_t>(1, (uint64_t)ctx->num_cus * 7 / 8);
    if (!knobs().screen_no_round && rows >= round) rows -= rows % round;
    return rows;
}
uint64_t oi_chunk_growth(uint32_t B) { return knobs().growth ? knobs().growth : (B <= 8 ? 16 : 8); }
uint64_t oi_chunk_end(uint64_t r, uint64_t chunk, uint64_t n, uint64_t max_chunk, uint64_t next_chunk) {
    uint64_t e = std::min(n, r + chunk);
    if (e < n && (n - e) * 4 <= (e - r) && n - r <= max_chunk) e = n;
    if (e < n && next_chunk >= max_chunk && n - e > max_chunk && n - r <= 2 * max_chunk) e = n - max_chunk;
    return e;
}

struct Chunk { uint64_t r, e; };
std::vector<Chunk> chunk_schedule(uint64_t n, uint64_t first, uint64_t growth, uint64_t max_chunk, bool stretch_first) {
    std::vector<Chunk> out;
    uint64_t chunk = first, r = 0;
    while (r < n) {
        if (chunk > max_chunk) chunk = max_chunk;
        const uint64_t e = oi_chunk_end(r, chunk, n, max_chunk, r == 0 && !stretch_first ? 0 : chunk * growth);
        out.push_back(Chunk{r, e});
        r = e;
        chunk *= growth;
    }
    return out;
}

struct Search {
    oi_index *idx; oi_ctx *ctx;
    const float *qv; const uint32_t *qt, *qo;
    uint32_t B, depth;
    float *cos_s; uint32_t *cos_d, *cos_c;
    float *bm_s; uint32_t *bm_d, *bm_c;
    const uint4 *filt; const uint2 *attrs;
};
enum class CosRoute { none, bf16, exact, screen_f32, screen_copy, screen_i8 };

struct Plan {
    CosRoute cos = CosRoute::none;
    int bm25 = BM25_STREAM;
    uint64_t cos_stride = 0, pf_stride = 0, pf_slack = 0;
    uint32_t pf_carry = 4096;
    bool spec = false;
    std::vector<Chunk> screen_chunks;
    bool overlap = false, late_fork = false, tail_fork = false;
    uint32_t screen_wgs = 0;
};
bool screened(CosRoute c) { return c == CosRoute::screen_f32 || c == CosRoute::screen_copy || c == CosRoute::screen_i8; }

Plan plan_search(const Search &s) {
    oi_index *idx = s.idx; oi_ctx *ctx = s.ctx;
    const Knobs &K = knobs();
    const uint64_t n = idx->n_docs;
    const uint32_t B = s.B, depth = s.depth, carry_cap = OI_MAX_DEPTH;
    Plan p;
    const int mode = ctx->cosine_mode;
    const bool want_copy = mode != OI_COSINE_SCREEN_STREAM && (idx->screen_copy.p != nullptr || (mode == OI_COSINE_SCREEN_COPY && !idx->is_view));
    const bool screen = (mode == OI_COSINE_SCREEN || mode == OI_COSINE_SCREEN_COPY || mode == OI_COSINE_SCREEN_STREAM) &&
                        oi_index_screenable(idx) && (B > 8 || (want_copy && !K.small_gemv)) && !K.exact_only;
    if (!s.cos_s) p.cos = CosRoute::none;
    else if (idx->rows_bf16) p.cos = CosRoute::bf16;
    else if (!screen) p.cos = CosRoute::exact;
    else if (!want_copy) p.cos = s.filt ? CosRoute::exact : CosRoute::screen_f32;
    else if (B > 8 && idx->screen_copy.p && idx->screen_i8.p) p.cos = CosRoute::screen_i8;
    else p.cos = CosRoute::screen_copy;
    p.bm25 = bm25_mode_of(idx);
    if (p.bm25 == BM25_SCAN && !(idx->fwd_terms.p && idx->total_tokens > 0)) p.bm25 = BM25_STREAM;
    if (s.filt) p.bm25 = BM25_STREAM;
    const uint64_t slack = (idx->rows_bf16 ? 128ull : 32ull) * ((uint64_t)ctx->num_cus + 1);
    const uint64_t budget = (idx->rows_bf16 ? (8ull << 30) : (13ull << 28)) / 8 / B;
    p.cos_stride = std::min<uint64_t>(carry_cap + n + slack, std::max<uint64_t>(std::min<uint64_t>(1ull << 24, budget), carry_cap + 4 * slack));
    p.pf_carry = p.cos == CosRoute::screen_i8 ? OI_I8_CARRY : 4096;
    p.pf_slack = 128ull * ((uint64_t)ctx->num_cus + 1);
    p.pf_stride = std::min<uint64_t>(p.pf_carry + n + p.pf_slack, std::max<uint64_t>(std::min<uint64_t>(1ull << 24, budget), p.pf_carry + 4 * p.pf_slack));
    uint64_t first = oi_screen_first_chunk_rows(ctx, depth), growth = oi_chunk_growth(B);
    const uint64_t pool_max = p.pf_stride - p.pf_carry - p.pf_slack;
    if (screened(p.cos) && B > 8 && !s.filt) {
        oi_spec_take_failure(ctx);
        p.spec = ctx->speculate && !K.no_spec && !ctx->use_graphs;
        if (p.spec && ctx->spec_skip) { --ctx->spec_skip; p.spec = false; }
        if (p.spec && !ctx->spec_fail_host) {
            if (hipHostMalloc(reinterpret_cast<void **>(&ctx->spec_fail_host), 64, hipHostMallocDefault) == hipSuccess) *ctx->spec_fail_host = 0;
            else { (void)hipGetLastError(); ctx->spec_fail_host = nullptr; p.spec = false; }
        }
        if (p.spec && n) {
            const uint64_t first_short = std::min<uint64_t>(n, std::max<uint64_t>(std::max<uint64_t>(8192, 8ull * depth), first / K.spec_first_div));
            if (n - first_short <= pool_max && 2 * ((3ull * depth * first_short + n - 1) / n + 12) <= depth) {
                growth = K.spec_growth;
                first = first_short;
            } else if (2 * ((3ull * depth * std::min<uint64_t>(n, first) + n - 1) / n + 12) <= depth) growth = K.spec_growth;
        }
    }
    if (screened(p.cos)) p.screen_chunks = chunk_schedule(n, first, growth, pool_max, false);
    if (s.cos_s && s.bm_s && !ctx->side_stream && !ctx->side_stream_failed && ctx->overlap_legs && !K.no_overlap) {
        if (hipStreamCreateWithFlags(&ctx->side_stream, hipStreamNonBlocking) != hipSuccess) { ctx->side_stream = nullptr; ctx->side_stream_failed = true; }
    }
    p.overlap = s.cos_s && s.bm_s && ctx->side_stream && ctx->ev_fork && ctx->ev_join && ctx->overlap_legs && !K.no_overlap;
    p.late_fork = p.overlap && !K.bm25_early && B > 8 && !p.screen_chunks.empty() &&
                  p.screen_chunks.back().e - p.screen_chunks.back().r >= (512u << 10);
    p.tail_fork = p.late_fork && p.cos == CosRoute::screen_i8 && !K.bm25_beside_last;
    if (p.cos == CosRoute::screen_i8 && !idx->is_view && (!p.overlap || p.tail_fork) && !K.screen_i8_narrow)
        p.screen_wgs = (uint32_t)std::max(1, ctx->num_cus);
    return p;
}

int bm25_stream(const Search &s, const PoolView &bm) {
    oi_index *idx = s.idx; oi_ctx *ctx = s.ctx;
    const uint32_t B = s.B, depth = s.depth, carry_cap = OI_MAX_DEPTH, nb = idx->n_blocks;
    if (nb == 0 || idx->n_postings == 0) {
        OI_HIP_CHECK(hipMemsetAsync(s.bm_c, 0, sizeof(uint32_t) * B, ctx->stream));
        return OI_OK;
    }
    const bool floors = idx->impact_floor.p != nullptr && !knobs().bm25_two_phase && !s.filt;
    const uint32_t first = floors ? nb : nb > 48 ? std::max<uint32_t>(8, nb / knobs().bm25_first_div) : nb;
    const uint32_t cap1 = oi_bm25_stream_seg_cap(depth, !floors), cap2 = oi_bm25_stream_seg_cap(depth, false);
    const uint64_t sstride = (uint64_t)carry_cap + std::max<uint64_t>((uint64_t)first * cap1, (uint64_t)nb * cap2);
    uint64_t pass = (2ull << 30) / 8 / sstride;
    pass = std::max<uint64_t>(1, std::min<uint64_t>(pass, std::min<uint32_t>(B, oi_bm25_stream_pass_queries())));
    DevBuf &sp = ctx->buf("pool_bm_stream"), &sc = ctx->buf("pool_bm_stream_state");
    OI_CHECK(sp.ensure(sizeof(uint64_t) * (size_t)pass * sstride));
    const size_t swords = (size_t)pass * (2 + nb);
    OI_CHECK(sc.ensure(sizeof(uint32_t) * swords));
    for (uint32_t q0 = 0; q0 < B; q0 += (uint32_t)pass) {
        const uint32_t nq = std::min<uint32_t>((uint32_t)pass, B - q0);
        uint32_t *w = sc.as<uint32_t>();
        OI_CHECK(oi_launch_bm25_plan(idx, s.qt, s.qo, q0, nq, w, swords, depth, (uint32_t)pass, (uint32_t)pass, floors));
        PoolView W1{sp.as<uint64_t>(), w, w + 2 * (size_t)pass, w + pass, sstride, carry_cap, cap1, first, nb, bm.overflow, s.filt, s.attrs};
        OI_CHECK(oi_launch_bm25_stream(idx, s.qt, s.qo, q0, nq, depth, W1, 0, first));
        PoolView W2 = W1;
        if (first < nb) {
            OI_CHECK(oi_launch_select(ctx, W1, nq, depth, true, nullptr, nullptr, nullptr, depth));
            W2.seg_cap = cap2; W2.n_segs = nb;
            OI_CHECK(oi_launch_bm25_stream(idx, s.qt, s.qo, q0, nq, depth, W2, first, nb));
        }
        OI_CHECK(oi_launch_select(ctx, W2, nq, depth, false, s.bm_s + (size_t)q0 * depth, s.bm_d + (size_t)q0 * depth, s.bm_c + q0, depth));
    }
    return OI_OK;
}
int bm25_wave(const Search &s, const PoolView &bm) {
    oi_index *idx = s.idx; oi_ctx *ctx = s.ctx;
    const uint32_t B = s.B, depth = s.depth, carry_cap = OI_MAX_DEPTH, nb = idx->n_blocks;
    if (nb == 0 || idx->n_postings == 0) {
        OI_HIP_CHECK(hipMemsetAsync(s.bm_c, 0, sizeof(uint32_t) * B, ctx->stream));
        return OI_OK;
    }
    const uint64_t wstride = (uint64_t)carry_cap + (uint64_t)nb * OI_BM25_BLOCK_DOCS;
    uint64_t pass = (6ull << 30) / 8 / wstride;
    pass = std::max<uint64_t>(1, std::min<uint64_t>(pass, std::min<uint32_t>(B, oi_bm25_wave_pass_queries())));
    DevBuf &wp = ctx->buf("pool_bm_wave"), &wc = ctx->buf("pool_bm_wave_state");
    OI_CHECK(wp.ensure(sizeof(uint64_t) * (size_t)pass * wstride));
    const size_t wwords = (size_t)pass * (2 + nb);
    OI_CHECK(wc.ensure(sizeof(uint32_t) * wwords));
    const uint32_t first = nb > 16 ? std::max<uint32_t>(8, nb / 8) : nb;
    for (uint32_t q0 = 0; q0 < B; q0 += (uint32_t)pass) {
        const uint32_t nq = std::min<uint32_t>((uint32_t)pass, B - q0);
        OI_HIP_CHECK(hipMemsetAsync(wc.p, 0, sizeof(uint32_t) * wwords, ctx->stream));
        uint32_t *w = wc.as<uint32_t>();
        PoolView W{wp.as<uint64_t>(), w, w + 2 * (size_t)pass, w + pass, wstride, carry_cap, OI_BM25_BLOCK_DOCS, nb, nb, bm.overflow};
        OI_CHECK(oi_launch_bm25_wave(idx, s.qt, s.qo, q0, nq, W, 0, first));
        if (first < nb) {
            OI_CHECK(oi_launch_select(ctx, W, nq, depth, true, nullptr, nullptr, nullptr, depth));
            OI_CHECK(oi_launch_bm25_wave(idx, s.qt, s.qo, q0, nq, W, first, nb));
        }
        OI_CHECK(oi_launch_select(ctx, W, nq, depth, false, s.bm_s + (size_t)q0 * depth, s.bm_d + (size_t)q0 * depth, s.bm_c + q0, depth));
    }
    return OI_OK;
}
int bm25_taat(const Search &s, const PoolView &bm) {
    const uint32_t nb = s.idx->n_blocks;
    const uint32_t first = nb > 16 ? std::max<uint32_t>(8, nb / 8) : nb;
    OI_CHECK(oi_launch_bm25(s.idx, s.qt, s.qo, s.B, s.depth, bm, 0, first));
    if (first < nb) {
        OI_CHECK(oi_launch_select(s.ctx, bm, s.B, s.depth, true, nullptr, nullptr, nullptr, s.depth));
        OI_CHECK(oi_launch_bm25(s.idx, s.qt, s.qo, s.B, s.depth, bm, first, nb));
    }
    return oi_launch_select(s.ctx, bm, s.B, s.depth, false, s.bm_s, s.bm_d, s.bm_c, s.depth);
}
int bm25_scan(const Search &s, const PoolView &bm) {
    oi_index *idx = s.idx; oi_ctx *ctx = s.ctx;
    const uint64_t n = idx->n_docs;
    const uint32_t B = s.B, depth = s.depth, carry_cap = OI_MAX_DEPTH;
    const uint32_t segs = 2u * (uint32_t)ctx->num_cus;
    const uint64_t sslack = 1024ull * (segs + 1);
    uint64_t sstride = carry_cap + std::min<uint64_t>(n, 1ull << 23) + sslack;
    const uint64_t sbudget = (4ull << 30) / 8 / B;
    if (sstride > sbudget) sstride = std::max<uint64_t>(sbudget, carry_cap + 4 * sslack);
    DevBuf &sp = ctx->buf("pool_bm_scan"), &sc = ctx->buf("pool_bm_scan_state");
    OI_CHECK(sp.ensure(sizeof(uint64_t) * (size_t)B * sstride));
    const size_t swords = (size_t)B * (2 + segs);
    OI_CHECK(sc.ensure(sizeof(uint32_t) * swords));
    OI_HIP_CHECK(hipMemsetAsync(sc.p, 0, sizeof(uint32_t) * swords, ctx->stream));
    uint32_t *w = sc.as<uint32_t>();
    PoolView SP{sp.as<uint64_t>(), w, w + 2 * (size_t)B, w + B, sstride, carry_cap, 0, 0, segs, bm.overflow};
    const uint64_t max_chunk = sstride - carry_cap - sslack;
    const uint32_t pass = oi_bm25_scan_pass_queries(idx->max_query_terms);
    for (uint32_t q0 = 0; q0 < B; q0 += pass) {
        const uint32_t nq = std::min(pass, B - q0);
        PoolView V = SP;
        V.carry_cnt += q0; V.tau_keys += q0;
        uint64_t r = 0, chunk = std::max<uint64_t>(n / 8, 65536);
        while (r < n) {
            if (chunk > max_chunk) chunk = max_chunk;
            const uint64_t e = std::min(n, r + chunk);
            oi_bm25_scan_geometry(ctx, e - r, &V.n_segs, &V.seg_cap);
            SP.n_segs = V.n_segs; SP.seg_cap = V.seg_cap;
            OI_CHECK(oi_launch_bm25_scan(idx, s.qt, s.qo, q0, nq, r, e, idx->avgdl, r == 0, SP));
            const bool last = e == n;
            PoolView S2 = SP;
            S2.keys += (uint64_t)q0 * sstride; S2.carry_cnt += q0; S2.tau_keys += q0; S2.seg_cnt += (uint64_t)q0 * segs;
            OI_CHECK(oi_launch_select(ctx, S2, nq, depth, !last, last ? s.bm_s + (size_t)q0 * depth : nullptr,
                                      last ? s.bm_d + (size_t)q0 * depth : nullptr, last ? s.bm_c + q0 : nullptr, depth));
            r = e;
            chunk = n;
        }
    }
    return OI_OK;
}
int bm25_leg(const Search &s, const Plan &p, const PoolView &bm) {
    OI_REQUIRE(s.idx->finalized, "search: index not finalized");
    return p.bm25 == BM25_TAAT ? bm25_taat(s, bm) : p.bm25 == BM25_SCAN ? bm25_scan(s, bm) : p.bm25 == BM25_WAVE ? bm25_wave(s, bm)
                                                                                                               : bm25_stream(s, bm);
}
int fork_bm25(const Search &s, const Plan &p, const PoolView &bm) {
    oi_ctx *ctx = s.ctx;
    hipStream_t st = ctx->stream;
    OI_HIP_CHECK(hipStreamWaitEvent(ctx->side_stream, ctx->ev_fork, 0));
    ctx->stream = ctx->side_stream;
    const int rc = bm25_leg(s, p, bm);
    ctx->stream = st;
    if (rc != OI_OK) { (void)hipStreamSynchronize(ctx->side_stream); return rc; }
    OI_HIP_CHECK(hipEventRecord(ctx->ev_join, ctx->side_stream));
    return OI_OK;
}

int cosine_bf16(const Search &s, const Plan &p, PoolView C) {
    oi_index *idx = s.idx;
    C.filt = s.filt; C.attrs = s.attrs;
    const uint64_t bslack = 128ull * ((uint64_t)s.ctx->num_cus + 1), room = p.cos_stride - OI_MAX_DEPTH;
    const uint64_t max_chunk = room > bslack ? room - bslack : 0;
    if (max_chunk == 0) { oi_set_error("search: cosine pool too small"); return OI_ERR_STATE; }
    for (const Chunk &c : chunk_schedule(idx->n_docs, oi_first_chunk_rows(s.depth), oi_chunk_growth(s.B), max_chunk, true)) {
        OI_CHECK(oi_launch_cosine_bf16_chunk(s.ctx, idx->rows_bf16, c.r, c.e, idx->dim, s.qv, s.B, idx->doc_id_base, C));
        const bool last = c.e == idx->n_docs;
        OI_CHECK(oi_launch_select(s.ctx, C, s.B, s.depth, !last, last ? s.cos_s : nullptr,
                                  last ? s.cos_d : nullptr, last ? s.cos_c : nullptr, s.depth));
    }
    return OI_OK;
}
int cosine_exact(const Search &s, PoolView X, const float *q, uint32_t Bp, uint64_t max_chunk, const uint32_t *gate, uint32_t *screen_tau) {
    oi_index *idx = s.idx;
    SelectExtra ex; ex.run_gate = gate;
    if (screen_tau) X.tau_keys = screen_tau;
    X.filt = s.filt; X.attrs = s.attrs;
    const uint64_t first = gate ? max_chunk : oi_first_chunk_rows(s.depth);
    for (const Chunk &c : chunk_schedule(idx->n_docs, first, oi_chunk_growth(s.B), max_chunk, true)) {
        OI_CHECK(oi_launch_cosine_chunk(s.ctx, idx->rows, c.r, c.e, idx->dim, q, s.B, Bp, idx->doc_id_base, X));
        const bool last = c.e == idx->n_docs;
        OI_CHECK(oi_launch_select(s.ctx, X, s.B, s.depth, !last, last ? s.cos_s : nullptr,
                                  last ? s.cos_d : nullptr, last ? s.cos_c : nullptr, s.depth, gate ? &ex : nullptr));
    }
    return OI_OK;
}
int cosine_screen(const Search &s, const Plan &p, const Pools &P, uint32_t *w, const float *q, uint32_t Bp, uint64_t max_chunk) {
    oi_index *idx = s.idx; oi_ctx *ctx = s.ctx;
    const uint64_t n = idx->n_docs;
    const uint32_t B = s.B, depth = s.depth, dim = idx->dim;
    const bool i8 = p.cos == CosRoute::screen_i8, copy = p.cos != CosRoute::screen_f32;
    const uint32_t segs = (uint32_t)ctx->num_cus;
    DevBuf &pk = ctx->buf("pool_cos"), &rk = ctx->buf("screen_rescored"), &qb = ctx->buf("screen_q_bf16");
    const uint32_t rs_cap = p.pf_carry + OI_LONG_ROWS_MAX;
    OI_CHECK(rk.ensure(sizeof(uint64_t) * (size_t)B * rs_cap));
    const uint32_t n_padded = (B + 31u) & ~31u;
    OI_CHECK(qb.ensure(sizeof(uint16_t) * (size_t)(n_padded + 64) * dim));
    uint32_t *pf_cnt = w, *pf_tau = w + B, *rs_cnt = w + 2 * (size_t)B;
    float *eps2 = reinterpret_cast<float *>(w + 3 * (size_t)B);
    uint32_t *gate = w + 4 * (size_t)B, *pf_seg = gate + 4;
    uint32_t *spec_tau = pf_seg + (size_t)B * segs, *spec_max = spec_tau + B;
    PoolView PF{pk.as<uint64_t>(), pf_cnt, pf_seg, pf_tau, p.pf_stride, p.pf_carry, 0, 0, segs, P.cos.overflow, s.filt, s.attrs};
    PoolView RS{rk.as<uint64_t>(), rs_cnt, pf_seg, nullptr, rs_cap, rs_cap, 0, 0, segs, P.cos.overflow, s.filt, s.attrs};
    static const bool stage_split = oi_ablation_env("OI_STAGE_SPLIT") != nullptr;
    if (!i8 || stage_split) OI_CHECK(oi_launch_screen_stage(ctx, s.qv, B, dim, idx->max_row_norm.as<uint32_t>(), qb.as<uint16_t>(), eps2, gate));
    SelectExtra mx; mx.eps2 = eps2; mx.margin_gate = gate;
    if (idx->n_long) { mx.skip_bitmap = idx->long_bitmap.as<uint32_t>(); mx.skip_base = idx->doc_id_base; }
    if (copy && !idx->screen_copy.p) {
        OI_CHECK(idx->screen_copy.ensure(sizeof(uint16_t) * (size_t)n * dim + 64));
        OI_CHECK(oi_launch_make_screen_copy(ctx, idx->rows, n, dim, idx->screen_copy.as<uint16_t>()));
    }
    int8_t *qi8 = nullptr; float *qf8 = nullptr;
    SelectExtra m8 = mx;
    if (i8) {
        DevBuf &qs = ctx->buf("screen_q_i8"), &cb = ctx->buf("screen_i8_cand");
        const size_t qi8_bytes = ((2 * (size_t)n_padded * dim) + 255) & ~(size_t)255;
        OI_CHECK(qs.ensure(qi8_bytes + sizeof(float) * 4 * (size_t)n_padded));
        OI_CHECK(cb.ensure(sizeof(uint64_t) * (size_t)B * OI_I8_CARRY));
        qi8 = reinterpret_cast<int8_t *>(qs.p);
        qf8 = reinterpret_cast<float *>(reinterpret_cast<unsigned char *>(qs.p) + qi8_bytes);
        OI_CHECK(oi_launch_screen_stage_i8(ctx, s.qv, B, dim, idx->max_row_norm.as<uint32_t>(), idx->screen_i8.as<uint8_t>(), n,
                                           qi8, qf8, gate, stage_split ? nullptr : qb.as<uint16_t>(), stage_split ? nullptr : eps2));
        m8.eps2 = qf8 + 3 * (size_t)n_padded; m8.row_qn = qf8 + (size_t)n_padded; m8.row_cq = qf8 + 2 * (size_t)n_padded;
        m8.cand = cb.as<uint64_t>(); m8.cand_cap = OI_I8_CARRY;
        m8.row_meta = reinterpret_cast<const float *>(idx->screen_i8.as<uint8_t>() + oi_screen_i8_meta_offset(n, dim));
        m8.meta_base = idx->doc_id_base;
    }
    bool spec_next = false, spec_any = false;
    for (size_t i = 0; i < p.screen_chunks.size(); ++i) {
        const uint64_t r = p.screen_chunks[i].r, e = p.screen_chunks[i].e;
        const bool last = i + 1 == p.screen_chunks.size();
        if (p.late_fork && !p.tail_fork && last) OI_HIP_CHECK(hipEventRecord(ctx->ev_fork, ctx->stream));
        uint32_t *const proven_tau = PF.tau_keys;
        if (spec_next) PF.tau_keys = spec_tau;
        const int rc_screen = i8 ? oi_launch_cosine_screen_i8_chunk(ctx, idx->screen_i8.as<uint8_t>(), n, r, e, dim, qi8, qf8, B, idx->doc_id_base, PF, p.screen_wgs)
                              : copy ? oi_launch_cosine_screen_copy_chunk(ctx, idx->screen_copy.as<uint16_t>(), r, e, dim, qb.as<uint16_t>(), B, idx->doc_id_base, PF)
                                     : oi_launch_cosine_screen_chunk(ctx, idx->rows, r, e, dim, qb.as<uint16_t>(), B, idx->doc_id_base, PF);
        PF.tau_keys = proven_tau;
        OI_CHECK(rc_screen);
        ctx->last_screen_wgs = i ? std::max(ctx->last_screen_wgs, PF.n_segs) : PF.n_segs;
        if (p.tail_fork && last) OI_HIP_CHECK(hipEventRecord(ctx->ev_fork, ctx->stream));
        if (p.late_fork && last) OI_CHECK(fork_bm25(s, p, P.bm));
        static const int spec_kernel = oi_ablation_env("OI_SPEC_KERNEL") ? atoi(oi_ablation_env("OI_SPEC_KERNEL")) : 0;
        const uint64_t rank = (3ull * depth * e + n - 1) / n + 12;
        const bool spec_here = p.spec && !last && 2 * rank <= depth;
        SelectExtra sx = i8 ? m8 : mx;
        if (spec_here && spec_kernel != 1) { sx.spec_rank = (uint32_t)rank; sx.spec_tau = spec_tau; sx.spec_max = spec_max; }
        uint32_t *chk = nullptr;
        if (spec_here && spec_kernel == 2) {
            DevBuf &cw = ctx->buf("spec_check");
            OI_CHECK(cw.ensure(sizeof(uint32_t) * 2 * (size_t)B));
            chk = cw.as<uint32_t>();
            OI_HIP_CHECK(hipMemcpyAsync(chk + B, spec_max, sizeof(uint32_t) * B, hipMemcpyDeviceToDevice, ctx->stream));
        }
        OI_CHECK(oi_launch_select(ctx, PF, B, depth, true, nullptr, nullptr, nullptr, depth, &sx));
        spec_next = false;
        if (spec_here) {
            if (spec_kernel != 1) { ProfScope ps(ctx, "spec"); }
            if (spec_kernel == 1) OI_CHECK(oi_launch_spec_threshold(ctx, PF, B, (uint32_t)rank, sx.eps2, spec_tau, spec_max));
            if (chk) {
                OI_CHECK(oi_launch_spec_threshold(ctx, PF, B, (uint32_t)rank, sx.eps2, chk, chk + B));
                OI_CHECK(oi_launch_spec_compare(ctx, B, spec_tau, spec_max, chk, chk + B));
            }
            spec_next = spec_any = true;
        }
    }
    if (spec_any) ++ctx->spec_searches;
    PoolView PR = PF;
    if (i8) {
        OI_CHECK(oi_launch_rescreen_bf16(ctx, idx->screen_copy.as<uint16_t>(), n, dim, idx->doc_id_base, qb.as<uint16_t>(), B, PF));
        PoolView PB = PF; PB.tau_keys = nullptr; PB.n_segs = 0;
        OI_CHECK(oi_launch_select(ctx, PB, B, depth, true, nullptr, nullptr, nullptr, depth, &mx));
        PR.carry_cap = 4096;
    }
    OI_CHECK(oi_launch_rescore(ctx, idx->rows, n, dim, idx->doc_id_base, s.qv, B, PR, RS,
                               idx->n_long ? idx->long_list.as<uint32_t>() : nullptr, idx->n_long,
                               spec_any ? spec_max : nullptr, pf_tau, gate, ctx->spec_fail_host));
    RS.n_segs = 0;
    OI_CHECK(oi_launch_select(ctx, RS, B, depth, false, s.cos_s, s.cos_d, s.cos_c, depth));
    ctx->run_gate = ctx->last_screen_gate = gate;
    const int rc = cosine_exact(s, P.cos, q, Bp, max_chunk, gate, pf_tau);
    ctx->run_gate = nullptr;
    return rc;
}

int cosine_leg(const Search &s, const Plan &p, const Pools &P, uint32_t *screen_state) {
    if (p.cos == CosRoute::none) return OI_OK;
    if (p.cos == CosRoute::bf16) return cosine_bf16(s, p, P.cos);
    oi_index *idx = s.idx; oi_ctx *ctx = s.ctx;
    OI_REQUIRE(idx->rows, "search: embeddings not set");
    const uint32_t Bp = oi_cosine_query_padding(s.B);
    const float *q = s.qv;
    if (Bp != s.B) {
        DevBuf &qp = ctx->buf("q_padded");
        OI_CHECK(qp.ensure(sizeof(float) * (size_t)Bp * idx->dim));
        OI_HIP_CHECK(hipMemsetAsync(qp.p, 0, sizeof(float) * (size_t)Bp * idx->dim, ctx->stream));
        OI_HIP_CHECK(hipMemcpyAsync(qp.p, s.qv, sizeof(float) * (size_t)s.B * idx->dim, hipMemcpyDeviceToDevice, ctx->stream));
        q = qp.as<float>();
    }
    const uint64_t max_chunk = oi_cosine_max_chunk_rows(ctx, idx->dim, s.B, p.cos_stride, OI_MAX_DEPTH);
    if (max_chunk == 0) { oi_set_error("search: cosine pool too small"); return OI_ERR_STATE; }
    if (p.cos == CosRoute::exact) {
        ctx->last_screen_gate = nullptr;
        return cosine_exact(s, P.cos, q, Bp, max_chunk, nullptr, nullptr);
    }
    return cosine_screen(s, p, P, screen_state, q, Bp, max_chunk);
}

}

void oi_spec_take_failure(oi_ctx *ctx) {
    if (!ctx->spec_fail_host || !*ctx->spec_fail_host) return;
    *ctx->spec_fail_host = 0; ++ctx->spec_failures;
    ctx->spec_backoff = ctx->spec_backoff ? std::min(1024u, 2 * ctx->spec_backoff) : 16u;
    ctx->spec_skip = ctx->spec_backoff;
}
int search_lists_device(oi_index *idx, const float *d_qv, const uint32_t *d_qt, const uint32_t *d_qo, uint32_t B, uint32_t depth,
                        float *cos_s, uint32_t *cos_d, uint32_t *cos_c, float *bm_s, uint32_t *bm_d, uint32_t *bm_c,
                        const uint4 *d_filt, const uint2 *d_attrs) {
    oi_ctx *ctx = idx->ctx;
    const Search s{idx, ctx, d_qv, d_qt, d_qo, B, depth, cos_s, cos_d, cos_c, bm_s, bm_d, bm_c, d_filt, d_attrs};
    const Plan p = plan_search(s);
    Pools P;
    const size_t screen_words = (size_t)B * (6 + (size_t)ctx->num_cus) + 4;
    uint32_t *screen_state = nullptr;
    OI_CHECK(prepare_pools(ctx, B, std::max<uint64_t>(p.cos_stride, idx->rows_bf16 ? 0ull : p.pf_stride), p.cos_stride, OI_MAX_DEPTH,
                           p.bm25 == BM25_TAAT ? idx->n_blocks : 0, depth, &P, screen_words, &screen_state));
    if (p.overlap && !p.late_fork) {
        OI_HIP_CHECK(hipEventRecord(ctx->ev_fork, ctx->stream));
        OI_CHECK(fork_bm25(s, p, P.bm));
    }
    const int rc = cosine_leg(s, p, P, screen_state);
    if (rc != OI_OK) {
        if (p.overlap) (void)hipStreamSynchronize(ctx->side_stream);
        return rc;
    }
    if (p.overlap) OI_HIP_CHECK(hipStreamWaitEvent(ctx->stream, ctx->ev_join, 0));
    else if (bm_s) OI_CHECK(bm25_leg(s, p, P.bm));
    return OI_OK;
}
```

openintel_amd/csrc/select.hip:

```cpp
#include "oi_device.h"
#include "oi_internal.h"

#define SEL_THREADS 1024
#define SEL_MAX 1024

struct SelArgs {
    uint64_t *pools;
    uint32_t *carry_cnt, *seg_cnt, *tau_keys, *overflow;
    uint64_t pool_stride;
    uint32_t carry_cap, seg_cap, n_segs, seg_cnt_stride, k, out_stride;
    int compact;
    float *out_scores;
    uint32_t *out_docs, *out_counts;
    const float *eps2, *row_meta, *row_qn, *row_cq;
    const uint32_t *run_gate, *skip;
    uint32_t *margin_gate, *spec_tau, *spec_max;
    uint64_t *cand;
    uint32_t skip_base, cand_cap, meta_base, spec_rank;
};

__device__ void bitonic_sort_desc(uint64_t *a, uint32_t P) {
    const uint32_t tid = threadIdx.x;
    for (uint32_t size = 2; size <= P; size <<= 1) {
        for (uint32_t stride = size >> 1; stride > 0; stride >>= 1) {
            for (uint32_t t = tid; t < (P >> 1); t += SEL_THREADS) {
                uint32_t lo = 2 * t - (t & (stride - 1));
                uint32_t hi = lo + stride;
                bool desc = ((lo & size) == 0);
                uint64_t x = a[lo], y = a[hi];
                if ((x < y) == desc) { a[lo] = y; a[hi] = x; }
            }
            __syncthreads();
        }
    }
}

#define SEL_MAX_SEGS 4096
#define SEL_KPT_MAX 32
#ifdef OI_ABLATION
__device__ int sel_dbg_on;
__device__ unsigned long long sel_dbg_t[16];
#define SEL_STAMP(i) do { if (sel_dbg_on && blockIdx.x == 0 && threadIdx.x == 0) sel_dbg_t[i] = __builtin_readcyclecounter(); } while (0)
#else
#define SEL_STAMP(i) do { } while (0)
#endif
#define SEL_CAND 4096

struct SelRowMargin {
    const float *meta;
    uint32_t base;
    float qn, cq;
};
__device__ __forceinline__ float sel_row_e(const SelRowMargin &rm, uint64_t kv) {
    return rm.meta[2 * (uint64_t)(oi_rank_key_doc(kv) - rm.base) + 1];
}
__device__ __forceinline__ bool sel_row_test(const SelRowMargin &rm, uint64_t kv, float e, float edge, float eps2) {
    const float u = oi_rank_key_score(kv) + 2.002f * (e * rm.qn + rm.cq);
    return u >= edge - 9.5367431640625e-07f * (fabsf(edge) + eps2);
}
__device__ __forceinline__ bool sel_row_keep(const SelRowMargin &rm, uint64_t kv, float edge, float eps2) {
    if (!rm.meta) return true;
    return sel_row_test(rm, kv, sel_row_e(rm, kv), edge, eps2);
}

__device__ __forceinline__ void sel_spec_words(bool have, uint32_t rth_key, float eps2, uint32_t tau, uint32_t *spec_tau, uint32_t *spec_max) {
    if (!have) { *spec_tau = tau; return; }
    const float s = oi_key_f32(rth_key) - eps2;
    const uint32_t T = s == s ? oi_f32_key(s) : 0u;
    const uint32_t st = T > tau ? T : tau;
    *spec_tau = st;
    if (st > tau && st > *spec_max) *spec_max = st;
}

struct SelRadix {
    uint32_t hist[256];
    uint32_t kk, bin_cnt;
    uint64_t prefix;
};
struct SelShared {
    SelRadix rx;
    uint32_t hist2k[2048];
    uint32_t seg_off[SEL_MAX_SEGS + 1];
    uint32_t wave_tot[SEL_THREADS / 64];
    uint32_t cnt, n_samples;
    unsigned long long min_key;
};

__device__ __forceinline__ void sel_hist_add(uint32_t *hist, bool active, uint32_t digit) {
    const uint32_t lane = threadIdx.x & 63;
#pragma unroll
    for (int r = 0; r < 2; ++r) {
        const unsigned long long m = __ballot(active);
        if (!m) return;
        const uint32_t leader = (uint32_t)__builtin_ctzll(m);
        const uint32_t d0 = (uint32_t)__shfl((int)digit, (int)leader, OI_WAVE);
        const unsigned long long same = __ballot(active && digit == d0);
        if (lane == leader) atomicAdd(&hist[d0], (uint32_t)__popcll(same));
        active = active && digit != d0;
    }
    if (active) atomicAdd(&hist[digit], 1u);
}

__device__ __forceinline__ void sel_append(uint64_t *dst, uint32_t *count, uint32_t cap, bool take, uint64_t key) {
    const unsigned long long m = __ballot(take);
    if (!m) return;
    const uint32_t lane = threadIdx.x & 63, leader = (uint32_t)__builtin_ctzll(m);
    uint32_t base = 0;
    if (lane == leader) base = atomicAdd(count, (uint32_t)__popcll(m));
    base = (uint32_t)__shfl((int)base, (int)leader, OI_WAVE);
    const uint32_t pos = base + (uint32_t)__popcll(m & ((1ull << lane) - 1ull));
    if (take && pos < cap) dst[pos] = key;
}

__device__ __forceinline__ void sel_hist_add_w(uint32_t *hist, bool active, uint32_t digit, uint32_t weight) {
    const uint32_t lane = threadIdx.x & 63;
#pragma unroll
    for (int r = 0; r < 2; ++r) {
        const unsigned long long m = __ballot(active);
        if (!m) return;
        const uint32_t leader = (uint32_t)__builtin_ctzll(m);
        const uint32_t d0 = (uint32_t)__builtin_amdgcn_readlane((int)digit, (int)leader);
        const bool same = active && digit == d0;
        const uint32_t sum = (uint32_t)__builtin_amdgcn_readlane((int)oi_wave_incl_scan(same ? weight : 0u), 63);
        if (lane == leader) atomicAdd(&hist[d0], sum);
        active = active && !same;
    }
    if (active) atomicAdd(&hist[digit], weight);
}

__device__ __forceinline__ void sel_min_key(const uint64_t *a, uint32_t m, unsigned long long *min_key) {
    unsigned long long lo = ~0ull;
    for (uint32_t i = threadIdx.x; i < m; i += SEL_THREADS) lo = a[i] < lo ? a[i] : lo;
#pragma unroll
    for (int o = 32; o > 0; o >>= 1) {
        const unsigned long long v = __shfl_xor(lo, o, OI_WAVE);
        lo = v < lo ? v : lo;
    }
    if ((threadIdx.x & 63) == 0 && lo != ~0ull) atomicMin(min_key, lo);
}

template <class FE>
__device__ __forceinline__ void sel_threshold(FE &&for_each, uint32_t kk_in, SelRadix &rx, int &shift_out, uint64_t &prefix_out) {
    const uint32_t tid = threadIdx.x;
    if (tid == 0) { rx.prefix = 0; rx.kk = kk_in; }
    int shift = 56;
    for (;; shift -= 8) {
        if (tid < 256) rx.hist[tid] = 0;
        __syncthreads();
        const uint64_t prefix = rx.prefix;
        const bool top = shift == 56;
        for_each([&](bool valid, uint64_t kv) {
            sel_hist_add(rx.hist, valid && (top || (kv >> ((shift + 8) & 63)) == prefix), (uint32_t)(kv >> shift) & 255u);
        });
        __syncthreads();
        if (tid < 64) {
            const uint32_t kk = rx.kk;
            uint32_t mine = 0;
            for (int i = 0; i < 4; ++i) mine += rx.hist[255 - (tid * 4 + i)];
            uint32_t incl = mine;
#pragma unroll
            for (int o = 1; o < 64; o <<= 1) {
                const uint32_t v = __shfl_up(incl, o, OI_WAVE);
                if ((int)tid >= o) incl += v;
            }
            const unsigned long long ball = __ballot(incl >= kk);
            const uint32_t owner = ball ? (uint32_t)__builtin_ctzll(ball) : 63u;
            if (tid == owner) {
                uint32_t cum = incl - mine;
                int d = 255 - (int)(tid * 4);
                for (int i = 0; i < 3; ++i, --d) {
                    const uint32_t c = rx.hist[d];
                    if (cum + c >= kk) break;
                    cum += c;
                }
                rx.prefix = (prefix << 8) | (uint64_t)d;
                rx.kk = kk - cum;
                rx.bin_cnt = rx.hist[d];
            }
        }
        __syncthreads();
        if (rx.bin_cnt == 1 || shift == 0) break;
    }
    shift_out = shift;
    prefix_out = rx.prefix;
    __syncthreads();
}

__device__ __forceinline__ void sel_rank_bin2k(SelShared &sh, uint32_t kk, int pass) {
    const uint32_t tid = threadIdx.x;
    {
        uint32_t v = sh.hist2k[2 * tid] + sh.hist2k[2 * tid + 1];
        v += (uint32_t)__builtin_amdgcn_update_dpp(0, (int)v, 0x111, 0xf, 0xf, false);
        v += (uint32_t)__builtin_amdgcn_update_dpp(0, (int)v, 0x112, 0xf, 0xf, false);
        v += (uint32_t)__builtin_amdgcn_update_dpp(0, (int)v, 0x114, 0xf, 0xf, false);
        v += (uint32_t)__builtin_amdgcn_update_dpp(0, (int)v, 0x118, 0xf, 0xf, false);
        if ((tid & 15u) == 15u) sh.rx.hist[tid >> 4] = v;
    }
    __syncthreads();
    if (tid < 64) {
        const uint32_t x = sh.rx.hist[63u - tid];
        const uint32_t incl = oi_wave_incl_scan(x);
        const unsigned long long ball = __ballot(incl >= kk);
        if (!ball) {
            if (tid == 0) sh.rx.bin_cnt = 0xFFFFFFFFu;
        } else {
            const uint32_t l1 = (uint32_t)__builtin_ctzll(ball), sb = 63u - l1;
            const uint32_t kk2 = kk - (uint32_t)__builtin_amdgcn_readlane((int)(incl - x), (int)l1);
            const uint32_t y = tid < 32u ? sh.hist2k[32u * sb + 31u - tid] : 0u;
            const uint32_t incl2 = oi_wave_incl_scan(y);
            const unsigned long long ball2 = __ballot(incl2 >= kk2);
            const uint32_t l2 = ball2 ? (uint32_t)__builtin_ctzll(ball2) : 31u;
            const uint32_t above = (uint32_t)__builtin_amdgcn_readlane((int)(incl2 - y), (int)l2);
            if (tid == 0) {
                sh.rx.prefix = (uint64_t)(32u * sb + 31u - l2);
                sh.rx.kk = kk2 - above;
                sh.rx.bin_cnt = 1u;
#ifdef OI_ABLATION
                if (sel_dbg_on > 1) {
                    uint32_t cum = 0; int dd = 2047;
                    for (; dd >= 0; --dd) { if (cum + sh.hist2k[dd] >= kk) break; cum += sh.hist2k[dd]; }
                    if ((uint32_t)dd != (uint32_t)sh.rx.prefix || kk - cum != sh.rx.kk)
                        printf("MISMATCH q=%u pass=%d kk=%u: walk (%d, %u) super-bin (%u, %u) sb=%u l1=%u kk2=%u l2=%u\n", blockIdx.x, pass, kk, dd, kk - cum,
                               (uint32_t)sh.rx.prefix, sh.rx.kk, sb, l1, kk2, l2);
                }
#endif
            }
        }
    }
    __syncthreads();
}

template <class FE>
__device__ __forceinline__ void sel_hist_leading(FE &&for_each, SelShared &sh) {
    uint32_t run_d = 0, run_c = 0;
    for_each([&](bool valid, uint64_t kv) {
        if (valid) {
            const uint32_t d = (uint32_t)(kv >> 53);
            if (run_c && d != run_d) { atomicAdd(&sh.hist2k[run_d], run_c); run_c = 0; }
            run_d = d;
            ++run_c;
        }
    });
    sel_hist_add_w(sh.hist2k, run_c != 0u, run_d, run_c);
}

template <class FE>
__device__ __forceinline__ uint32_t sel_rth_score_key(FE &&for_each, uint32_t r, SelShared &sh) {
    const uint32_t tid = threadIdx.x;
    uint32_t kk = r, pfx = 0;
#pragma unroll
    for (int pass = 0; pass < 3; ++pass) {
        const int shift = pass == 0 ? 21 : pass == 1 ? 10 : 0, bits = pass == 2 ? 10 : 11;
        sh.hist2k[tid] = 0;
        sh.hist2k[tid + SEL_THREADS] = 0;
        __syncthreads();
        if (pass == 0) {
            sel_hist_leading(for_each, sh);
        } else {
            for_each([&](bool valid, uint64_t kv) {
                const uint32_t sk = (uint32_t)(kv >> 32);
                if (valid && (sk >> (shift + bits)) == pfx) atomicAdd(&sh.hist2k[(sk >> shift) & ((1u << bits) - 1u)], 1u);
            });
        }
        __syncthreads();
        sel_rank_bin2k(sh, kk, 2 + pass);
        const uint32_t d = sh.rx.bin_cnt != 0xFFFFFFFFu ? (uint32_t)sh.rx.prefix : 0u;
        kk = sh.rx.kk;
        __syncthreads();
        pfx = (pfx << bits) | d;
    }
    return pfx;
}
__device__ __forceinline__ uint32_t sel_rth_score_key_of(const uint64_t *a, uint32_t m, uint32_t r, SelShared &sh) {
    const uint32_t tid = threadIdx.x;
    return sel_rth_score_key([&](auto &&f) {
        for (uint32_t i0 = 0; i0 < m; i0 += SEL_THREADS) f(i0 + tid < m, a[i0 + tid < m ? i0 + tid : 0]);
    }, r, sh);
}

__device__ __forceinline__ void sel_finish(const SelArgs &a, uint32_t q, uint64_t *pool, uint32_t *segc, uint64_t *sel, uint32_t m,
                                           unsigned long long *min_key) {
    const uint32_t tid = threadIdx.x;
    if (a.out_scores) {
        uint32_t P = 2;
        while (P < m) P <<= 1;
        for (uint32_t i = m + tid; i < P; i += SEL_THREADS) sel[i] = 0;
        __syncthreads();
        bitonic_sort_desc(sel, P);
        for (uint32_t i = tid; i < m; i += SEL_THREADS) {
            const uint64_t key = sel[i];
            a.out_scores[(uint64_t)q * a.out_stride + i] = oi_rank_key_score(key);
            a.out_docs[(uint64_t)q * a.out_stride + i] = oi_rank_key_doc(key);
        }
        if (tid == 0) { a.out_counts[q] = m; *min_key = m ? sel[m - 1] : 0; }
    } else {
        sel_min_key(sel, m, min_key);
    }
    __syncthreads();
    if (a.compact) {
        for (uint32_t i = tid; i < m; i += SEL_THREADS) pool[i] = sel[i];
        for (uint32_t sg = tid; sg < a.n_segs; sg += SEL_THREADS) segc[sg] = 0;
        if (tid == 0) {
            a.carry_cnt[q] = m;
            if (m == a.k && a.tau_keys && !a.eps2) {
                const uint32_t t = (uint32_t)(*min_key >> 32);
                if (t > a.tau_keys[q]) a.tau_keys[q] = t;
            }
        }
    }
}

struct SelFlat {
    const uint64_t *pool;
    const uint32_t *seg_off;
    uint32_t n, c0, carry_cap, seg_cap, n_segs, steps;
};
struct SelCursor {
    uint32_t sg, lo, hi;
};
__device__ __forceinline__ SelCursor sel_seek(const SelFlat &K, uint32_t i) {
    const uint32_t e = i < K.c0 ? 0u : i - K.c0;
    uint32_t lo = 0, hi = K.n_segs;
    for (uint32_t s = 0; s < K.steps; ++s) {
        const uint32_t mid = (lo + hi) >> 1;
        const bool up = K.seg_off[mid] <= e;
        lo = up ? mid : lo;
        hi = up ? hi : mid;
    }
    SelCursor c;
    c.sg = lo; c.lo = K.seg_off[lo]; c.hi = K.seg_off[lo + 1];
    return c;
}
__device__ __forceinline__ uint64_t sel_at(const SelFlat &K, SelCursor &c, uint32_t i) {
    if (i < K.c0) return i;
    const uint32_t e = i - K.c0;
    while (e >= c.hi) {
        ++c.sg;
        c.lo = c.hi;
        c.hi = K.seg_off[c.sg + 1];
    }
    return (uint64_t)K.carry_cap + (uint64_t)c.sg * K.seg_cap + (e - c.lo);
}

struct SelMargin {
    float eps2;
    const uint32_t *skip;
    uint32_t skip_base;
    uint64_t *cand;
    uint32_t cap;
    uint64_t *carry;
    uint32_t spec_rank;
    SelRowMargin rows;
};
struct SelResult {
    uint32_t m;
    bool in_cand, overflow, in_carry;
    uint32_t tau, spec_key;
};
__device__ __forceinline__ SelResult sel_margin_result(uint32_t c, uint32_t cap, uint32_t tau, bool in_carry) {
    return SelResult{c > cap ? cap : c, true, c > cap, in_carry, tau, 0u};
}

template <int KPT>
struct SelKeys {
    static constexpr int NR = KPT > 0 ? KPT : 1;
    const SelFlat &K;
    const uint32_t *const skip;
    const uint32_t skip_base;
    const uint32_t tid = threadIdx.x, lane = tid & 63, wv = tid >> 6, n = K.n;
    const uint32_t kpt = (n + SEL_THREADS - 1) / SEL_THREADS;
    const uint32_t first = wv * kpt * 64 + lane, last = n - 1;
    uint64_t key[NR];
    uint32_t dead = 0;

    __device__ __forceinline__ SelKeys(const SelFlat &K_, const SelMargin &M) : K(K_), skip(M.skip), skip_base(M.skip_base) {}
    __device__ __forceinline__ bool skipped(uint64_t kv) const {
        const uint32_t d = oi_rank_key_doc(kv) - skip_base;
        return (skip[d >> 5] >> (d & 31u)) & 1u;
    }
    __device__ __forceinline__ bool live(int j) const { return first + (uint32_t)j * 64 < n && !((dead >> j) & 1u); }
    __device__ __forceinline__ void load() {
        if constexpr (KPT > 0) {
            SelCursor cur = sel_seek(K, first < n ? first : last);
            uint64_t at = sel_at(K, cur, first < n ? first : last);
#pragma unroll
            for (int j = 0; j < KPT; ++j) {
                const uint32_t i = first + (uint32_t)j * 64;
                if ((uint32_t)j < kpt && i < n) at = sel_at(K, cur, i);
                key[j] = K.pool[at];
            }
            if (skip) {
#pragma unroll
                for (int j = 0; j < KPT; ++j)
                    if ((uint32_t)j < kpt && first + (uint32_t)j * 64 < n && skipped(key[j])) dead |= 1u << j;
            }
        }
    }
    template <class F>
    __device__ __forceinline__ void for_each(F &&f) const {
        if constexpr (KPT > 0) {
#pragma unroll
            for (int j = 0; j < KPT; ++j)
                if ((uint32_t)j < kpt) f(live(j), key[j]);
        } else {
            SelCursor cur = sel_seek(K, first < n ? first : last);
            uint64_t at = sel_at(K, cur, first < n ? first : last);
            for (uint32_t j0 = 0; j0 < kpt; j0 += 4) {
                uint64_t kx[4];
                bool ok[4];
#pragma unroll
                for (int u = 0; u < 4; ++u) {
                    const uint32_t i = first + (j0 + u) * 64;
                    ok[u] = j0 + u < kpt && i < n;
                    if (ok[u]) at = sel_at(K, cur, i);
                    kx[u] = K.pool[at];
                }
#pragma unroll
                for (int u = 0; u < 4; ++u) f(ok[u] && !(skip && skipped(kx[u])), kx[u]);
            }
        }
    }
};

template <int KPT>
__device__ __forceinline__ uint32_t sel_take_all(const SelKeys<KPT> &H, SelShared &sh, uint64_t *sel) {
    H.for_each([&](bool valid, uint64_t kv) { sel_append(sel, &sh.cnt, 2 * SEL_MAX, valid, kv); });
    __syncthreads();
    return H.skip ? sh.cnt : H.n;
}

template <int KPT>
__device__ __forceinline__ SelResult sel_margin_bins(const SelKeys<KPT> &H, uint32_t k, const SelMargin &M, SelShared &sh) {
    const uint32_t tid = H.tid, lane = H.lane, kpt = H.kpt;
    const float eps2 = M.eps2;
    SelResult R = {};
    uint32_t kk = k, pfx = 0;
#pragma unroll
    for (int pass = 0; pass < 2; ++pass) {
        const int shift = 53 - 11 * pass;
        sh.hist2k[tid] = 0;
        sh.hist2k[tid + SEL_THREADS] = 0;
        __syncthreads();
        if (pass == 0) {
            sel_hist_leading([&](auto &&f) { H.for_each(f); }, sh);
        } else {
            H.for_each([&](bool valid, uint64_t kv) {
                if (valid && (uint32_t)(kv >> 53) == pfx) atomicAdd(&sh.hist2k[(uint32_t)(kv >> shift) & 2047u], 1u);
            });
        }
        __syncthreads();
        sel_rank_bin2k(sh, kk, pass);
        const bool enough = sh.rx.bin_cnt != 0xFFFFFFFFu;
        const uint32_t d = (uint32_t)sh.rx.prefix;
        kk = sh.rx.kk;
        __syncthreads();
        if (!enough) return R;
        if (pass == 0) pfx = d;
        else pfx = (pfx << 11) | d;
        SEL_STAMP(3 + pass);
    }
    uint32_t tkey = pfx << 10;
    tkey = tkey < 0x007FFFFFu ? 0x007FFFFFu : tkey;
    const uint32_t t32 = eps2 < __builtin_inff() ? oi_f32_key(oi_key_f32(tkey) - eps2) : 0u;
    uint32_t mine = 0;
    const float edge = oi_key_f32(tkey);
    auto keep = [&](bool valid, uint64_t kv) { return valid && (uint32_t)(kv >> 32) >= t32 && sel_row_keep(M.rows, kv, edge, eps2); };
    uint32_t verdict = 0;
    if constexpr (KPT > 0) {
#pragma unroll
        for (int j = 0; j < KPT; ++j)
            if ((uint32_t)j < kpt && H.live(j) && (uint32_t)(H.key[j] >> 32) >= t32) verdict |= 1u << j;
        if (M.rows.meta) {
            constexpr int G = KPT < 8 ? KPT : 8;
#pragma unroll
            for (int j0 = 0; j0 < KPT; j0 += G) {
                if ((uint32_t)j0 < kpt) {
                    float e[G];
#pragma unroll
                    for (int u = 0; u < G; ++u) e[u] = (verdict >> (j0 + u)) & 1u ? sel_row_e(M.rows, H.key[j0 + u]) : 0.f;
#pragma unroll
                    for (int u = 0; u < G; ++u)
                        if (((verdict >> (j0 + u)) & 1u) && !sel_row_test(M.rows, H.key[j0 + u], e[u], edge, eps2)) verdict &= ~(1u << (j0 + u));
                }
            }
        }
        mine = (uint32_t)__popc(verdict);
    } else {
        H.for_each([&](bool valid, uint64_t kv) { mine += keep(valid, kv) ? 1u : 0u; });
    }
    const uint32_t incl = oi_wave_incl_scan(mine);
    const uint32_t tot = (uint32_t)__builtin_amdgcn_readlane((int)incl, 63);
    uint32_t base = 0;
    if (lane == 0 && tot) base = atomicAdd(&sh.cnt, tot);
    uint32_t pos = (uint32_t)__builtin_amdgcn_readfirstlane((int)base) + incl - mine;
    uint32_t stored = 0;
    if constexpr (KPT > 0) {
#pragma unroll
        for (int j = 0; j < KPT; ++j) {
            if ((verdict >> j) & 1u) {
                if (pos < M.cap) { M.carry[pos] = H.key[j]; stored |= 1u << j; }
                ++pos;
            }
        }
    } else {
        H.for_each([&](bool valid, uint64_t kv) {
            if (keep(valid, kv)) {
                if (pos < M.cap) M.cand[pos] = kv;
                ++pos;
            }
        });
    }
    __syncthreads();
    R = sel_margin_result(sh.cnt, M.cap, t32, KPT > 0);
    SEL_STAMP(5);
    if constexpr (KPT > 0) {
        if (M.spec_rank && R.m >= M.spec_rank)
            R.spec_key = sel_rth_score_key([&](auto &&f) {
#pragma unroll
                for (int j = 0; j < KPT; ++j)
                    if ((uint32_t)j < kpt) f((stored >> j) & 1u, H.key[j]);
            }, M.spec_rank, sh);
    }
    return R;
}

template <int KPT>
__device__ __forceinline__ bool sel_sampled_cut(const SelKeys<KPT> &H, uint32_t k, SelShared &sh, uint64_t *sel, uint64_t *cand) {
    const uint32_t tid = H.tid, lane = H.lane, kpt = H.kpt, first = H.first, last = H.last, n = H.n;
    int shift;
    uint64_t prefix;
    const uint32_t js = lane % kpt, is = first + js * 64;
    bool sv = is < n;
    uint64_t sk;
    if constexpr (KPT > 0) {
        sk = H.key[0];
#pragma unroll
        for (int j = 1; j < KPT; ++j) sk = (uint32_t)j == js ? H.key[j] : sk;
        sv = sv && !((H.dead >> js) & 1u);
    } else {
        SelCursor cur = sel_seek(H.K, sv ? is : last);
        sk = H.K.pool[sel_at(H.K, cur, sv ? is : last)];
        sv = sv && !(H.skip && H.skipped(sk));
    }
    if (tid == 0) sh.n_samples = 0;
    __syncthreads();
    {
        const unsigned long long m = __ballot(sv);
        if (lane == 0 && m) atomicAdd(&sh.n_samples, (uint32_t)__popcll(m));
    }
    __syncthreads();
    const uint32_t ns = sh.n_samples;
    uint32_t r = (uint32_t)(((uint64_t)ns * (2 * k) + n - 1) / n) + 1;
    r = r > ns ? ns : r;
    sel_threshold([&](auto &&f) { f(sv, sk); }, r, sh.rx, shift, prefix);
    H.for_each([&](bool valid, uint64_t kv) { sel_append(cand, &sh.cnt, SEL_CAND, valid && (kv >> shift) >= prefix, kv); });
    __syncthreads();
    const uint32_t c = sh.cnt;
    __syncthreads();
    if (tid == 0) sh.cnt = 0;
    __syncthreads();
    if (c >= k && c <= SEL_CAND) {
        uint64_t ck[SEL_CAND / SEL_THREADS];
#pragma unroll
        for (int j = 0; j < SEL_CAND / SEL_THREADS; ++j) {
            const uint32_t i = (uint32_t)j * SEL_THREADS + tid;
            ck[j] = cand[i < c ? i : c - 1];
        }
        auto cand_each = [&](auto &&f) {
#pragma unroll
            for (int j = 0; j < SEL_CAND / SEL_THREADS; ++j)
                if ((uint32_t)j * SEL_THREADS < c) f((uint32_t)j * SEL_THREADS + tid < c, ck[j]);
        };
        if (c == k) {
            cand_each([&](bool valid, uint64_t kv) { sel_append(sel, &sh.cnt, SEL_MAX, valid, kv); });
        } else {
// ... 381 lines not shown
```

Measured before the change: 36480.

## Seed speculative screen threshold from an int8 sample pass before chunked screening

Adds a sampling pre-pass that scores a prefix of rows against all queries with int8 MFMA. It then ranks the sampled lower-bound keys per query to derive a speculative tau before the main chunked screen runs. A tighter early threshold is meant to reduce the candidates appended to pools and the selection work. In exchange it adds an extra kernel and a rank launch per batch, and relies on the speculation-failure fallback when the sampled threshold is too tight. The shared radix-select helpers move into a header so the new rank kernel can reuse them.

```diff
diff --git a/openintel_amd/csrc/api.hip b/openintel_amd/csrc/api.hip
--- a/openintel_amd/csrc/api.hip
+++ b/openintel_amd/csrc/api.hip
@@ -141,6 +141,11 @@
     if (strcmp(kernel_tag, "screen_width") == 0) {
         if (total_ms_out) *total_ms_out = (double)ctx->last_screen_wgs;
         if (launches_out) *launches_out = (uint64_t)ctx->num_cus;
+        return OI_OK;
+    }
+    if (strcmp(kernel_tag, "screen_sample") == 0) {
+        if (total_ms_out) *total_ms_out = (double)ctx->last_sample_rows;
+        if (launches_out) *launches_out = 0;
         return OI_OK;
     }
     if (strcmp(kernel_tag, "volume_state") == 0 || strcmp(kernel_tag, "summary_state") == 0 || strcmp(kernel_tag, "groups_state") == 0 ||
diff --git a/openintel_amd/csrc/cosine_screen_i8.hip b/openintel_amd/csrc/cosine_screen_i8.hip
--- a/openintel_amd/csrc/cosine_screen_i8.hip
+++ b/openintel_amd/csrc/cosine_screen_i8.hip
@@ -202,6 +202,9 @@
 #endif
 }
 
+__device__ __forceinline__ float i8s_screen_score(int S, float scale, float qa) { return (float)S * (scale * qa); }
+__device__ __forceinline__ float i8s_lower_bound(float sc, float er, float qn, float cq) { return sc - fmaf(er, qn, cq); }
+
 template <int D, int NQT, int NBUF, bool FILT>
 __global__ __launch_bounds__(256, 1) void cosine_i8_screen(
     const uint8_t *__restrict__ rows, const float *__restrict__ meta, uint64_t row_begin, uint64_t row_end,
@@ -439,7 +442,7 @@
                         const uint32_t bit = (uint32_t)__builtin_ctz(m), r = bit & 15u;
                         const bool t1 = NQT > 1 && bit >= 16u;
                         const uint32_t rit = (r & 3) + 8 * (r >> 2) + 4 * lh;
-                        const float low = cap_sc - fmaf(cap_er, t1 ? qn[NQT - 1] : qn[0], t1 ? cq[NQT - 1] : cq[0]);
+                        const float low = i8s_lower_bound(cap_sc, cap_er, t1 ? qn[NQT - 1] : qn[0], t1 ? cq[NQT - 1] : cq[0]);
                         const uint32_t below = __builtin_amdgcn_mbcnt_hi((uint32_t)(has >> 32), __builtin_amdgcn_mbcnt_lo((uint32_t)has, 0u));
                         const uint32_t idx = (st_head + st_n + below) & (OI_STAGE - 1);
                         stage_keys[idx] = oi_rank_key(low, doc_id_base + ((uint32_t)row0 + rit));
@@ -457,8 +460,8 @@
                     auto lower_key = [&](int t, uint32_t r) -> uint64_t {
                         const uint32_t rit = (r & 3) + 8 * (r >> 2) + 4 * lh;
                         const i8s_f32x2 md = *reinterpret_cast<const i8s_f32x2 *>(mt + rit * 8);
-                        const float sc = (float)S[16 * t + r] * (md[0] * qa[t]);
-                        return oi_rank_key(sc - fmaf(md[1], qn[t], cq[t]), doc_id_base + ((uint32_t)row0 + rit));
+                        const float sc = i8s_screen_score(S[16 * t + r], md[0], qa[t]);
+                        return oi_rank_key(i8s_lower_bound(sc, md[1], qn[t], cq[t]), doc_id_base + ((uint32_t)row0 + rit));
                     };
                     if (total <= OI_STAGE - OI_STAGE_FLUSH) {
                         uint32_t idx = st_head + st_n + incl - cnt;
@@ -567,6 +570,132 @@
     return OI_OK;
 }
 
+template <int D, int NQT>
+__global__ __launch_bounds__(256, 1) void i8s_sample_kernel(const uint8_t *__restrict__ rows, const float *__restrict__ meta, uint32_t m_rows,
+                                                            const int8_t *__restrict__ qhi, const int8_t *__restrict__ qlo,
+                                                            const float *__restrict__ qf, uint32_t qf_stride, uint32_t n_queries,
+                                                            const uint32_t *__restrict__ long_bitmap, uint32_t *__restrict__ keys,
+                                                            uint32_t key_stride) {
+    constexpr int KSTEPS = D / 32;
+    constexpr uint32_t PART = NQT * KSTEPS * 64;
+    static_assert(D % 32 == 0 && KSTEPS * 4 <= 128, "a tile's row fragments must fit the register file");
+    static_assert(2 * PART * 16 <= 160 * 1024, "LDS");
+    extern __shared__ __attribute__((aligned(1024))) unsigned char smem[];
+    OI_CLAIM_WHOLE_SIMD();
+    const uint32_t tid = threadIdx.x, lane = tid & 63;
+    const uint32_t w = __builtin_amdgcn_readfirstlane(tid >> 6);
+    const uint32_t li = lane & 31, lh = lane >> 5;
+    const uint32_t row0 = (blockIdx.x * 4u + w) * I8S_TILE_ROWS;
+    const bool has_tile = row0 < m_rows;
+
+    const uint32_t arow = has_tile ? (row0 + li < m_rows ? row0 + li : m_rows - 1u) : 0u;
+    i8s_i32x4 a[KSTEPS];
+#pragma unroll
+    for (int s = 0; s < KSTEPS; ++s) a[s] = *reinterpret_cast<const i8s_i32x4 *>(rows + (uint64_t)arow * D + 32 * s + 16 * lh);
+    constexpr int NCP = 2 * PART / 256;
+    static_assert(NCP * 256 == 2 * PART, "whole trips of the workgroup");
+    i8s_i32x4 qv[NCP];
+#pragma unroll
+    for (int i = 0; i < NCP; ++i) {
+        const uint32_t c = tid + 256u * i, f = c % PART, t = f / (KSTEPS * 64), s = (f / 64) % KSTEPS, l = f % 64;
+        qv[i] = *reinterpret_cast<const i8s_i32x4 *>((c < PART ? qhi : qlo) + (uint64_t)(32 * t + (l & 31)) * D + 32 * s + 16 * (l >> 5));
+    }
+#pragma unroll
+    for (int i = 0; i < NCP; ++i) *reinterpret_cast<i8s_i32x4 *>(smem + (tid + 256u * i) * 16) = qv[i];
+    float4 md[4][2];
+#pragma unroll
+    for (int j = 0; j < 4; ++j) {
+        const float4 *mp = reinterpret_cast<const float4 *>(meta + 2 * (uint64_t)((has_tile ? row0 : 0u) + 8 * j + 4 * lh));
+        md[j][0] = mp[0];
+        md[j][1] = mp[1];
+    }
+    const uint32_t long_word = long_bitmap && has_tile ? long_bitmap[row0 >> 5] : 0u;
+    float qa[NQT], qn[NQT], cq[NQT];
+#pragma unroll
+    for (int t = 0; t < NQT; ++t) {
+        const uint32_t q = 32u * t + li;
+        const bool real = q < n_queries;
+        qa[t] = real ? qf[q] * 0.0078125f : 0.f;
+        qn[t] = real ? qf[qf_stride + q] : 0.f;
+        cq[t] = real ? qf[2 * qf_stride + q] : 0.f;
+    }
+    __syncthreads();
+    if (!has_tile) return;
+
+    i8s_i32x16 ah[NQT], al[NQT];
+#pragma unroll
+    for (int t = 0; t < NQT; ++t)
+#pragma unroll
+        for (int r = 0; r < 16; ++r) { ah[t][r] = 0; al[t][r] = 0; }
+#pragma unroll
+    for (int s = 0; s < KSTEPS; ++s)
+#pragma unroll
+        for (int t = 0; t < NQT; ++t) {
+            const unsigned char *frag = smem + ((t * KSTEPS + s) * 64 + lane) * 16;
+            const i8s_i32x4 bh = *reinterpret_cast<const i8s_i32x4 *>(frag), bl = *reinterpret_cast<const i8s_i32x4 *>(frag + PART * 16);
+            ah[t] = __builtin_amdgcn_mfma_i32_32x32x32_i8(a[s], bh, ah[t], 0, 0, 0);
+            al[t] = __builtin_amdgcn_mfma_i32_32x32x32_i8(a[s], bl, al[t], 0, 0, 0);
+        }
+#pragma unroll
+    for (int t = 0; t < NQT; ++t) {
+        const uint32_t q = 32u * t + li;
+        const bool real = q < n_queries;
+#pragma unroll
+        for (int j = 0; j < 4; ++j) {
+            const float scale[4] = {md[j][0].x, md[j][0].z, md[j][1].x, md[j][1].z};
+            const float er[4] = {md[j][0].y, md[j][0].w, md[j][1].y, md[j][1].w};
+            uint32_t k[4];
+#pragma unroll
+            for (int c = 0; c < 4; ++c) {
+                const uint32_t rit = (uint32_t)(c + 8 * j) + 4u * lh;
+                const float sc = i8s_screen_score(ah[t][4 * j + c] * 128 + al[t][4 * j + c], scale[c], qa[t]);
+                const bool keep = real && row0 + rit < m_rows && !((long_word >> rit) & 1u) && sc == sc;
+                k[c] = keep ? oi_f32_key(i8s_lower_bound(sc, er[c], qn[t], cq[t])) : 0u;
+            }
+            *reinterpret_cast<uint4 *>(keys + (uint64_t)q * key_stride + row0 + 8 * j + 4 * lh) = make_uint4(k[0], k[1], k[2], k[3]);
+        }
+    }
+}
+
+template <int D, int NQT>
+static int launch_i8_sample(oi_ctx *ctx, const uint8_t *rows, const float *meta, uint32_t m_rows, const int8_t *qhi, const int8_t *qlo,
+                            const float *qf, uint32_t qf_stride, uint32_t nq, const uint32_t *long_bitmap, uint32_t *keys, uint32_t key_stride) {
+    constexpr size_t smem = 2 * NQT * (D / 32) * 64 * 16;
+    OI_CHECK(oi_dyn_lds(ctx, reinterpret_cast<const void *>(i8s_sample_kernel<D, NQT>), smem));
+    const uint32_t tiles = (m_rows + I8S_TILE_ROWS - 1) / I8S_TILE_ROWS;
+    hipLaunchKernelGGL((i8s_sample_kernel<D, NQT>), dim3((tiles + 3) / 4), dim3(256), smem, ctx->stream, rows, meta, m_rows, qhi, qlo, qf,
+                       qf_stride, nq, long_bitmap, keys, key_stride);
+    OI_HIP_CHECK(hipGetLastError());
+    return OI_OK;
+}
+
+uint32_t oi_screen_i8_sample_stride(uint32_t m_rows) { return (m_rows + 31u) & ~31u; }
+
+int oi_launch_screen_i8_sample(oi_ctx *ctx, const uint8_t *i8_copy, uint64_t n_rows_total, uint32_t m_rows, uint32_t dim, const int8_t *qi8,
+                               const float *qf, uint32_t n_queries, const uint32_t *long_bitmap, uint32_t *keys) {
+    OI_REQUIRE(oi_cosine_screen_supported(dim), "cosine screen (int8 sample): dim %u not instantiated (384, 768)", dim);
+    OI_REQUIRE(m_rows <= n_rows_total, "cosine screen (int8 sample): rows past the copy");
+    if (m_rows == 0 || n_queries == 0) return OI_OK;
+    const float *meta = reinterpret_cast<const float *>(i8_copy + oi_screen_i8_meta_offset(n_rows_total, dim));
+    const uint32_t np = (n_queries + 31u) & ~31u, ks = oi_screen_i8_sample_stride(m_rows);
+    ProfScope pc(ctx, "cosine");
+    ProfScope ps(ctx, "sample");
+    for (uint32_t q0 = 0; q0 < n_queries; q0 += 64) {
+        const uint32_t nq_here = std::min(64u, n_queries - q0);
+        const int8_t *qhi = qi8 + (uint64_t)q0 * dim, *qlo = qi8 + ((uint64_t)np + q0) * dim;
+        uint32_t *kq = keys + (uint64_t)q0 * ks;
+        const bool two = nq_here > 32;
+        if (dim == 768) {
+            if (two) OI_CHECK((launch_i8_sample<768, 2>(ctx, i8_copy, meta, m_rows, qhi, qlo, qf + q0, np, nq_here, long_bitmap, kq, ks)));
+            else OI_CHECK((launch_i8_sample<768, 1>(ctx, i8_copy, meta, m_rows, qhi, qlo, qf + q0, np, nq_here, long_bitmap, kq, ks)));
+        } else {
+            if (two) OI_CHECK((launch_i8_sample<384, 2>(ctx, i8_copy, meta, m_rows, qhi, qlo, qf + q0, np, nq_here, long_bitmap, kq, ks)));
+            else OI_CHECK((launch_i8_sample<384, 1>(ctx, i8_copy, meta, m_rows, qhi, qlo, qf + q0, np, nq_here, long_bitmap, kq, ks)));
+        }
+    }
+    return OI_OK;
+}
+
 __device__ __forceinline__ float i8s_bf16_lo(uint32_t w) { return __uint_as_float(w << 16); }
 __device__ __forceinline__ float i8s_bf16_hi(uint32_t w) { return __uint_as_float(w & 0xFFFF0000u); }
 __global__ __launch_bounds__(256) void pf_rescreen_kernel(const uint16_t *__restrict__ copy, uint64_t n_rows, uint32_t dim,
diff --git a/openintel_amd/csrc/oi_internal.h b/openintel_amd/csrc/oi_internal.h
--- a/openintel_amd/csrc/oi_internal.h
+++ b/openintel_amd/csrc/oi_internal.h
@@ -111,6 +111,7 @@
     const uint32_t *run_gate = nullptr;
     const uint32_t *last_screen_gate = nullptr;
     uint32_t last_screen_wgs = 0;
+    uint32_t last_sample_rows = 0;
     std::map<std::string, std::vector<ProfSpan>> prof;
     std::vector<hipEvent_t> event_pool;
     bool use_graphs = false;
@@ -311,6 +312,11 @@
 int oi_launch_cosine_screen_i8_chunk(oi_ctx *ctx, const uint8_t *i8_copy, uint64_t n_rows_total, uint64_t row_begin, uint64_t row_end,
                                      uint32_t dim, const int8_t *qi8, const float *qf, uint32_t n_queries, uint32_t doc_id_base,
                                      PoolView &pool, uint32_t wgs = 0);
+uint32_t oi_screen_i8_sample_stride(uint32_t m_rows);
+int oi_launch_screen_i8_sample(oi_ctx *ctx, const uint8_t *i8_copy, uint64_t n_rows_total, uint32_t m_rows, uint32_t dim, const int8_t *qi8,
+                               const float *qf, uint32_t n_queries, const uint32_t *long_bitmap, uint32_t *keys);
+int oi_launch_sample_rank(oi_ctx *ctx, const uint32_t *keys, uint32_t stride, uint32_t m, uint32_t n_queries, uint32_t r, const float *eps2,
+                          const uint32_t *tau_keys, uint32_t *spec_tau, uint32_t *spec_max);
 int oi_launch_rescreen_bf16(oi_ctx *ctx, const uint16_t *copy_rows, uint64_t n_rows, uint32_t dim, uint32_t doc_id_base,
                             const uint16_t *q_bf16, uint32_t n_queries, const PoolView &pool);
 int oi_launch_cosine_screen_copy_chunk(oi_ctx *ctx, const uint16_t *copy_rows, uint64_t row_begin, uint64_t row_end, uint32_t dim,
diff --git a/openintel_amd/csrc/oi_select_rank.h b/openintel_amd/csrc/oi_select_rank.h
--- /dev/null
+++ b/openintel_amd/csrc/oi_select_rank.h
@@ -0,0 +1,136 @@
+#pragma once
+
+#include "oi_device.h"
+
+#ifndef SEL_THREADS
+#define SEL_THREADS 1024
+#endif
+#ifndef SEL_MAX_SEGS
+#define SEL_MAX_SEGS 4096
+#endif
+static_assert(SEL_THREADS == 1024 && SEL_MAX_SEGS == 4096, "sel_rank_bin2k and SelShared are laid out for 1024 threads and 4096 segments");
+
+__device__ __forceinline__ void sel_spec_words(bool have, uint32_t rth_key, float eps2, uint32_t tau, uint32_t *spec_tau, uint32_t *spec_max) {
+    if (!have) { *spec_tau = tau; return; }
+    const float s = oi_key_f32(rth_key) - eps2;
+    const uint32_t T = s == s ? oi_f32_key(s) : 0u;
+    const uint32_t st = T > tau ? T : tau;
+    *spec_tau = st;
+    if (st > tau && st > *spec_max) *spec_max = st;
+}
+
+struct SelRadix {
+    uint32_t hist[256];
+    uint32_t kk, bin_cnt;
+    uint64_t prefix;
+};
+struct SelShared {
+    SelRadix rx;
+    uint32_t hist2k[2048];
+    uint32_t seg_off[SEL_MAX_SEGS + 1];
+    uint32_t wave_tot[SEL_THREADS / 64];
+    uint32_t cnt, n_samples;
+    unsigned long long min_key;
+};
+
+__device__ __forceinline__ void sel_hist_add_w(uint32_t *hist, bool active, uint32_t digit, uint32_t weight) {
+    const uint32_t lane = threadIdx.x & 63;
+#pragma unroll
+    for (int r = 0; r < 2; ++r) {
+        const unsigned long long m = __ballot(active);
+        if (!m) return;
+        const uint32_t leader = (uint32_t)__builtin_ctzll(m);
+        const uint32_t d0 = (uint32_t)__builtin_amdgcn_readlane((int)digit, (int)leader);
+        const bool same = active && digit == d0;
+        const uint32_t sum = (uint32_t)__builtin_amdgcn_readlane((int)oi_wave_incl_scan(same ? weight : 0u), 63);
+        if (lane == leader) atomicAdd(&hist[d0], sum);
+        active = active && !same;
+    }
+    if (active) atomicAdd(&hist[digit], weight);
+}
+
+__device__ __forceinline__ void sel_rank_bin2k(SelShared &sh, uint32_t kk, int pass) {
+    const uint32_t tid = threadIdx.x;
+    {
+        uint32_t v = sh.hist2k[2 * tid] + sh.hist2k[2 * tid + 1];
+        v += (uint32_t)__builtin_amdgcn_update_dpp(0, (int)v, 0x111, 0xf, 0xf, false);
+        v += (uint32_t)__builtin_amdgcn_update_dpp(0, (int)v, 0x112, 0xf, 0xf, false);
+        v += (uint32_t)__builtin_amdgcn_update_dpp(0, (int)v, 0x114, 0xf, 0xf, false);
+        v += (uint32_t)__builtin_amdgcn_update_dpp(0, (int)v, 0x118, 0xf, 0xf, false);
+        if ((tid & 15u) == 15u) sh.rx.hist[tid >> 4] = v;
+    }
+    __syncthreads();
+    if (tid < 64) {
+        const uint32_t x = sh.rx.hist[63u - tid];
+        const uint32_t incl = oi_wave_incl_scan(x);
+        const unsigned long long ball = __ballot(incl >= kk);
+        if (!ball) {
+            if (tid == 0) sh.rx.bin_cnt = 0xFFFFFFFFu;
+        } else {
+            const uint32_t l1 = (uint32_t)__builtin_ctzll(ball), sb = 63u - l1;
+            const uint32_t kk2 = kk - (uint32_t)__builtin_amdgcn_readlane((int)(incl - x), (int)l1);
+            const uint32_t y = tid < 32u ? sh.hist2k[32u * sb + 31u - tid] : 0u;
+            const uint32_t incl2 = oi_wave_incl_scan(y);
+            const unsigned long long ball2 = __ballot(incl2 >= kk2);
+            const uint32_t l2 = ball2 ? (uint32_t)__builtin_ctzll(ball2) : 31u;
+            const uint32_t above = (uint32_t)__builtin_amdgcn_readlane((int)(incl2 - y), (int)l2);
+            if (tid == 0) {
+                sh.rx.prefix = (uint64_t)(32u * sb + 31u - l2);
+                sh.rx.kk = kk2 - above;
+                sh.rx.bin_cnt = 1u;
+#ifdef SEL_RANK_SELFCHECK
+                if (sel_dbg_on > 1) {
+                    uint32_t cum = 0; int dd = 2047;
+                    for (; dd >= 0; --dd) { if (cum + sh.hist2k[dd] >= kk) break; cum += sh.hist2k[dd]; }
+                    if ((uint32_t)dd != (uint32_t)sh.rx.prefix || kk - cum != sh.rx.kk)
+                        printf("MISMATCH q=%u pass=%d kk=%u: walk (%d, %u) super-bin (%u, %u) sb=%u l1=%u kk2=%u l2=%u\n", blockIdx.x, pass, kk, dd, kk - cum,
+                               (uint32_t)sh.rx.prefix, sh.rx.kk, sb, l1, kk2, l2);
+                }
+#endif
+            }
+        }
+    }
+    __syncthreads();
+}
+
+template <class FE>
+__device__ __forceinline__ void sel_hist_leading(FE &&for_each, SelShared &sh) {
+    uint32_t run_d = 0, run_c = 0;
+    for_each([&](bool valid, uint64_t kv) {
+        if (valid) {
+            const uint32_t d = (uint32_t)(kv >> 53);
+            if (run_c && d != run_d) { atomicAdd(&sh.hist2k[run_d], run_c); run_c = 0; }
+            run_d = d;
+            ++run_c;
+        }
+    });
+    sel_hist_add_w(sh.hist2k, run_c != 0u, run_d, run_c);
+}
+
+template <class FE>
+__device__ __forceinline__ uint32_t sel_rth_score_key(FE &&for_each, uint32_t r, SelShared &sh) {
+    const uint32_t tid = threadIdx.x;
+    uint32_t kk = r, pfx = 0;
+#pragma unroll
+    for (int pass = 0; pass < 3; ++pass) {
+        const int shift = pass == 0 ? 21 : pass == 1 ? 10 : 0, bits = pass == 2 ? 10 : 11;
+        sh.hist2k[tid] = 0;
+        sh.hist2k[tid + SEL_THREADS] = 0;
+        __syncthreads();
+        if (pass == 0) {
+            sel_hist_leading(for_each, sh);
+        } else {
+            for_each([&](bool valid, uint64_t kv) {
+                const uint32_t sk = (uint32_t)(kv >> 32);
+                if (valid && (sk >> (shift + bits)) == pfx) atomicAdd(&sh.hist2k[(sk >> shift) & ((1u << bits) - 1u)], 1u);
+            });
+        }
+        __syncthreads();
+        sel_rank_bin2k(sh, kk, 2 + pass);
+        const uint32_t d = sh.rx.bin_cnt != 0xFFFFFFFFu ? (uint32_t)sh.rx.prefix : 0u;
+        kk = sh.rx.kk;
+        __syncthreads();
+        pfx = (pfx << bits) | d;
+    }
+    return pfx;
+}
diff --git a/openintel_amd/csrc/sample_rank.hip b/openintel_amd/csrc/sample_rank.hip
--- /dev/null
+++ b/openintel_amd/csrc/sample_rank.hip
@@ -0,0 +1,39 @@
+#include "oi_internal.h"
+#include "oi_select_rank.h"
+
+#define SEL_KPT_MAX 32
+
+__global__ __launch_bounds__(SEL_THREADS) void sample_rank_kernel(const uint32_t *__restrict__ keys, uint32_t stride, uint32_t m, uint32_t r,
+                                                                  const float *__restrict__ eps2, const uint32_t *__restrict__ tau_keys,
+                                                                  uint32_t *spec_tau, uint32_t *spec_max) {
+    __shared__ SelShared sh;
+    const uint32_t q = blockIdx.x, tid = threadIdx.x;
+    const uint32_t *kq = keys + (uint64_t)q * stride;
+    const uint32_t kpt = (stride + SEL_THREADS - 1) / SEL_THREADS;
+    uint32_t key[SEL_KPT_MAX];
+#pragma unroll
+    for (int j = 0; j < SEL_KPT_MAX; ++j) {
+        const uint32_t i = (uint32_t)j * SEL_THREADS + tid;
+        key[j] = (uint32_t)j < kpt && i < stride ? kq[i] : 0u;
+    }
+    const bool have = m >= r;
+    uint32_t rth = 0;
+    if (have)
+        rth = sel_rth_score_key([&](auto &&f) {
+#pragma unroll
+            for (int j = 0; j < SEL_KPT_MAX; ++j)
+                if ((uint32_t)j < kpt) f((uint32_t)j * SEL_THREADS + tid < stride, (uint64_t)key[j] << 32);
+        }, r, sh);
+    if (tid == 0) sel_spec_words(have, rth, eps2[q], tau_keys[q], spec_tau + q, spec_max + q);
+}
+
+int oi_launch_sample_rank(oi_ctx *ctx, const uint32_t *keys, uint32_t stride, uint32_t m, uint32_t n_queries, uint32_t r, const float *eps2,
+                          const uint32_t *tau_keys, uint32_t *spec_tau, uint32_t *spec_max) {
+    if (n_queries == 0) return OI_OK;
+    OI_REQUIRE(r >= 1 && m <= stride && stride <= SEL_KPT_MAX * SEL_THREADS, "sample rank: %u keys of %u, rank %u", m, stride, r);
+    ProfScope pl(ctx, "select");
+    ProfScope ps(ctx, "spec");
+    hipLaunchKernelGGL(sample_rank_kernel, dim3(n_queries), dim3(SEL_THREADS), 0, ctx->stream, keys, stride, m, r, eps2, tau_keys, spec_tau, spec_max);
+    OI_HIP_CHECK(hipGetLastError());
+    return OI_OK;
+}
diff --git a/openintel_amd/csrc/search.hip b/openintel_amd/csrc/search.hip
--- a/openintel_amd/csrc/search.hip
+++ b/openintel_amd/csrc/search.hip
@@ -13,6 +13,7 @@
     uint32_t bm25_first_div = env_int("OI_BM25_FIRST_DIV", 8, 1);
     bool screen_no_round = env_set("OI_SCREEN_NO_ROUND"), no_spec = env_set("OI_NO_SPEC"), no_overlap = env_set("OI_NO_OVERLAP");
     bool bm25_beside_last = env_set("OI_BM25_BESIDE_LAST"), screen_i8_narrow = env_set("OI_SCREEN_I8_NARROW");
+    bool no_sample_pass = env_set("OI_NO_SAMPLE_PASS");
     bool bm25_early = env_set("OI_BM25_EARLY"), small_gemv = env_set("OI_SMALL_BATCH_GEMV"), bm25_two_phase = env_set("OI_BM25_TWO_PHASE");
     bool exact_only = env_set("OI_COSINE_V1") || env_set("OI_SELECT_V1");
 };
@@ -101,6 +102,7 @@
     uint32_t pf_carry = 4096;
     bool spec = false;
     std::vector<Chunk> screen_chunks;
+    uint32_t sample_rows = 0;
     bool overlap = false, late_fork = false, tail_fork = false;
     uint32_t screen_wgs = 0;
 };
@@ -150,6 +152,16 @@
         }
     }
     if (screened(p.cos)) p.screen_chunks = chunk_schedule(n, first, growth, pool_max, false);
+    if (p.cos == CosRoute::screen_i8 && p.spec && !K.no_sample_pass && p.screen_chunks.size() >= 2) {
+        const uint64_t m = p.screen_chunks[0].e;
+        const uint64_t key_words = (uint64_t)((B + 31u) & ~31u) * ((m + 31) & ~31ull);
+        if (2 * ((3ull * depth * m + n - 1) / n + 12) <= depth && p.screen_chunks[1].e <= pool_max && m <= (32u << 10) &&
+            key_words <= 2 * (uint64_t)B * p.pf_stride) {
+            p.sample_rows = (uint32_t)m;
+            p.screen_chunks.erase(p.screen_chunks.begin());
+            p.screen_chunks[0].r = 0;
+        }
+    }
     if (s.cos_s && s.bm_s && !ctx->side_stream && !ctx->side_stream_failed && ctx->overlap_legs && !K.no_overlap) {
         if (hipStreamCreateWithFlags(&ctx->side_stream, hipStreamNonBlocking) != hipSuccess) { ctx->side_stream = nullptr; ctx->side_stream_failed = true; }
     }
@@ -361,6 +373,17 @@
         m8.meta_base = idx->doc_id_base;
     }
     bool spec_next = false, spec_any = false;
+    if (p.sample_rows) {
+        const uint32_t ks = oi_screen_i8_sample_stride(p.sample_rows);
+        OI_REQUIRE(sizeof(uint32_t) * (size_t)n_padded * ks <= sizeof(uint64_t) * (size_t)B * p.pf_stride && pk.p,
+                   "search: the sample pass's keys do not fit the candidate pool");
+        uint32_t *sample_keys = pk.as<uint32_t>();
+        OI_CHECK(oi_launch_screen_i8_sample(ctx, idx->screen_i8.as<uint8_t>(), n, p.sample_rows, dim, qi8, qf8, B,
+                                            idx->n_long ? idx->long_bitmap.as<uint32_t>() : nullptr, sample_keys));
+        const uint64_t rank = (3ull * depth * p.sample_rows + n - 1) / n + 12;
+        OI_CHECK(oi_launch_sample_rank(ctx, sample_keys, ks, p.sample_rows, B, (uint32_t)rank, m8.eps2, pf_tau, spec_tau, spec_max));
+        spec_next = spec_any = true;
+    }
     for (size_t i = 0; i < p.screen_chunks.size(); ++i) {
         const uint64_t r = p.screen_chunks[i].r, e = p.screen_chunks[i].e;
         const bool last = i + 1 == p.screen_chunks.size();
@@ -455,6 +478,7 @@
     oi_ctx *ctx = idx->ctx;
     const Search s{idx, ctx, d_qv, d_qt, d_qo, B, depth, cos_s, cos_d, cos_c, bm_s, bm_d, bm_c, d_filt, d_attrs};
     const Plan p = plan_search(s);
+    ctx->last_sample_rows = p.sample_rows;
     Pools P;
     const size_t screen_words = (size_t)B * (6 + (size_t)ctx->num_cus) + 4;
     uint32_t *screen_state = nullptr;
diff --git a/openintel_amd/csrc/select.hip b/openintel_amd/csrc/select.hip
--- a/openintel_amd/csrc/select.hip
+++ b/openintel_amd/csrc/select.hip
@@ -2,6 +2,19 @@
 #include "oi_internal.h"
 
 #define SEL_THREADS 1024
+#define SEL_MAX_SEGS 4096
+#ifdef OI_ABLATION
+__device__ int sel_dbg_on;
+__device__ unsigned long long sel_dbg_t[16];
+#define SEL_STAMP(i) do { if (sel_dbg_on && blockIdx.x == 0 && threadIdx.x == 0) sel_dbg_t[i] = __builtin_readcyclecounter(); } while (0)
+#else
+#define SEL_STAMP(i) do { } while (0)
+#endif
+#ifdef OI_ABLATION
+#define SEL_RANK_SELFCHECK 1
+#endif
+#include "oi_select_rank.h"
+
 #define SEL_MAX 1024
 
 struct SelArgs {
@@ -35,15 +48,7 @@
     }
 }
 
-#define SEL_MAX_SEGS 4096
 #define SEL_KPT_MAX 32
-#ifdef OI_ABLATION
-__device__ int sel_dbg_on;
-__device__ unsigned long long sel_dbg_t[16];
-#define SEL_STAMP(i) do { if (sel_dbg_on && blockIdx.x == 0 && threadIdx.x == 0) sel_dbg_t[i] = __builtin_readcyclecounter(); } while (0)
-#else
-#define SEL_STAMP(i) do { } while (0)
-#endif
 #define SEL_CAND 4096
 
 struct SelRowMargin {
@@ -62,29 +67,6 @@
     if (!rm.meta) return true;
     return sel_row_test(rm, kv, sel_row_e(rm, kv), edge, eps2);
 }
-
-__device__ __forceinline__ void sel_spec_words(bool have, uint32_t rth_key, float eps2, uint32_t tau, uint32_t *spec_tau, uint32_t *spec_max) {
-    if (!have) { *spec_tau = tau; return; }
-    const float s = oi_key_f32(rth_key) - eps2;
-    const uint32_t T = s == s ? oi_f32_key(s) : 0u;
-    const uint32_t st = T > tau ? T : tau;
-    *spec_tau = st;
-    if (st > tau && st > *spec_max) *spec_max = st;
-}
-
-struct SelRadix {
-    uint32_t hist[256];
-    uint32_t kk, bin_cnt;
-    uint64_t prefix;
-};
-struct SelShared {
-    SelRadix rx;
-    uint32_t hist2k[2048];
-    uint32_t seg_off[SEL_MAX_SEGS + 1];
-    uint32_t wave_tot[SEL_THREADS / 64];
-    uint32_t cnt, n_samples;
-    unsigned long long min_key;
-};
 
 __device__ __forceinline__ void sel_hist_add(uint32_t *hist, bool active, uint32_t digit) {
     const uint32_t lane = threadIdx.x & 63;
@@ -110,22 +92,6 @@
     base = (uint32_t)__shfl((int)base, (int)leader, OI_WAVE);
     const uint32_t pos = base + (uint32_t)__popcll(m & ((1ull << lane) - 1ull));
     if (take && pos < cap) dst[pos] = key;
-}
-
-__device__ __forceinline__ void sel_hist_add_w(uint32_t *hist, bool active, uint32_t digit, uint32_t weight) {
-    const uint32_t lane = threadIdx.x & 63;
-#pragma unroll
-    for (int r = 0; r < 2; ++r) {
-        const unsigned long long m = __ballot(active);
-        if (!m) return;
-        const uint32_t leader = (uint32_t)__builtin_ctzll(m);
-        const uint32_t d0 = (uint32_t)__builtin_amdgcn_readlane((int)digit, (int)leader);
-        const bool same = active && digit == d0;
-        const uint32_t sum = (uint32_t)__builtin_amdgcn_readlane((int)oi_wave_incl_scan(same ? weight : 0u), 63);
-        if (lane == leader) atomicAdd(&hist[d0], sum);
-        active = active && !same;
-    }
-    if (active) atomicAdd(&hist[digit], weight);
 }
 
 __device__ __forceinline__ void sel_min_key(const uint64_t *a, uint32_t m, unsigned long long *min_key) {
@@ -186,91 +152,6 @@
     __syncthreads();
 }
 
-__device__ __forceinline__ void sel_rank_bin2k(SelShared &sh, uint32_t kk, int pass) {
-    const uint32_t tid = threadIdx.x;
-    {
-        uint32_t v = sh.hist2k[2 * tid] + sh.hist2k[2 * tid + 1];
-        v += (uint32_t)__builtin_amdgcn_update_dpp(0, (int)v, 0x111, 0xf, 0xf, false);
-        v += (uint32_t)__builtin_amdgcn_update_dpp(0, (int)v, 0x112, 0xf, 0xf, false);
-        v += (uint32_t)__builtin_amdgcn_update_dpp(0, (int)v, 0x114, 0xf, 0xf, false);
-        v += (uint32_t)__builtin_amdgcn_update_dpp(0, (int)v, 0x118, 0xf, 0xf, false);
-        if ((tid & 15u) == 15u) sh.rx.hist[tid >> 4] = v;
-    }
-    __syncthreads();
-    if (tid < 64) {
-        const uint32_t x = sh.rx.hist[63u - tid];
-        const uint32_t incl = oi_wave_incl_scan(x);
-        const unsigned long long ball = __ballot(incl >= kk);
-        if (!ball) {
-            if (tid == 0) sh.rx.bin_cnt = 0xFFFFFFFFu;
-        } else {
-            const uint32_t l1 = (uint32_t)__builtin_ctzll(ball), sb = 63u - l1;
-            const uint32_t kk2 = kk - (uint32_t)__builtin_amdgcn_readlane((int)(incl - x), (int)l1);
-            const uint32_t y = tid < 32u ? sh.hist2k[32u * sb + 31u - tid] : 0u;
-            const uint32_t incl2 = oi_wave_incl_scan(y);
-            const unsigned long long ball2 = __ballot(incl2 >= kk2);
-            const uint32_t l2 = ball2 ? (uint32_t)__builtin_ctzll(ball2) : 31u;
-            const uint32_t above = (uint32_t)__builtin_amdgcn_readlane((int)(incl2 - y), (int)l2);
-            if (tid == 0) {
-                sh.rx.prefix = (uint64_t)(32u * sb + 31u - l2);
-                sh.rx.kk = kk2 - above;
-                sh.rx.bin_cnt = 1u;
-#ifdef OI_ABLATION
-                if (sel_dbg_on > 1) {
-                    uint32_t cum = 0; int dd = 2047;
-                    for (; dd >= 0; --dd) { if (cum + sh.hist2k[dd] >= kk) break; cum += sh.hist2k[dd]; }
-                    if ((uint32_t)dd != (uint32_t)sh.rx.prefix || kk - cum != sh.rx.kk)
-                        printf("MISMATCH q=%u pass=%d kk=%u: walk (%d, %u) super-bin (%u, %u) sb=%u l1=%u kk2=%u l2=%u\n", blockIdx.x, pass, kk, dd, kk - cum,
-                               (uint32_t)sh.rx.prefix, sh.rx.kk, sb, l1, kk2, l2);
-                }
-#endif
-            }
-        }
-    }
-    __syncthreads();
-}
-
-template <class FE>
-__device__ __forceinline__ void sel_hist_leading(FE &&for_each, SelShared &sh) {
-    uint32_t run_d = 0, run_c = 0;
-    for_each([&](bool valid, uint64_t kv) {
-        if (valid) {
-            const uint32_t d = (uint32_t)(kv >> 53);
-            if (run_c && d != run_d) { atomicAdd(&sh.hist2k[run_d], run_c); run_c = 0; }
-            run_d = d;
-            ++run_c;
-        }
-    });
-    sel_hist_add_w(sh.hist2k, run_c != 0u, run_d, run_c);
-}
-
-template <class FE>
-__device__ __forceinline__ uint32_t sel_rth_score_key(FE &&for_each, uint32_t r, SelShared &sh) {
-    const uint32_t tid = threadIdx.x;
-    uint32_t kk = r, pfx = 0;
-#pragma unroll
-    for (int pass = 0; pass < 3; ++pass) {
-        const int shift = pass == 0 ? 21 : pass == 1 ? 10 : 0, bits = pass == 2 ? 10 : 11;
-        sh.hist2k[tid] = 0;
-        sh.hist2k[tid + SEL_THREADS] = 0;
-        __syncthreads();
-        if (pass == 0) {
-            sel_hist_leading(for_each, sh);
-        } else {
-            for_each([&](bool valid, uint64_t kv) {
-                const uint32_t sk = (uint32_t)(kv >> 32);
-                if (valid && (sk >> (shift + bits)) == pfx) atomicAdd(&sh.hist2k[(sk >> shift) & ((1u << bits) - 1u)], 1u);
-            });
-        }
-        __syncthreads();
-        sel_rank_bin2k(sh, kk, 2 + pass);
-        const uint32_t d = sh.rx.bin_cnt != 0xFFFFFFFFu ? (uint32_t)sh.rx.prefix : 0u;
-        kk = sh.rx.kk;
-        __syncthreads();
-        pfx = (pfx << bits) | d;
-    }
-    return pfx;
-}
 __device__ __forceinline__ uint32_t sel_rth_score_key_of(const uint64_t *a, uint32_t m, uint32_t r, SelShared &sh) {
     const uint32_t tid = threadIdx.x;
     return sel_rth_score_key([&](auto &&f) {
```

After: 37570 (median of 6 runs). +3.0%, better.
